# mohammadasim98/mv-ldm

Measured on AMD Instinct MI355X. Metric: denoised views/sec @ 256x256, 4 views, 50 DDIM steps, higher is better.
Workload: dtype bf16

## Files before the change

include/mvldm.h:

```cpp
#ifndef MVLDM_H
#define MVLDM_H

#include <stddef.h>
#include <stdint.h>

#ifdef __cplusplus
extern "C" {
#endif

#define MVLDM_ABI_VERSION 7

typedef void* mvldm_stream_t;

enum { MVLDM_F32 = 0, MVLDM_BF16 = 1, MVLDM_F16 = 2 };
enum { MVLDM_OK = 0, MVLDM_ERR_ARG = -1, MVLDM_ERR_HIP = -2, MVLDM_ERR_UNSUPPORTED = -3 };

enum { MVLDM_EPI_NONE = 0, MVLDM_EPI_SILU = 1, MVLDM_EPI_GEGLU = 2, MVLDM_EPI_GELU = 3  };
enum { MVLDM_ELT_COPY = 0, MVLDM_ELT_SILU = 1, MVLDM_ELT_GELU = 2 };

int mvldm_abi_version(void);
int mvldm_build_flags(void);
const char* mvldm_last_error(void);
int mvldm_device_info(int* cu_count, size_t* hbm_bytes, char* arch, int arch_len);

typedef struct mvldm_igemm_desc {
    const void* src0;
    const void* src1;
    const void* weight;
    const float* bias;
    const float* row_bias;
    const void* residual;
    void* dst;
    float* workspace;
    int32_t c0, c1;
    int32_t n_img, h_in, w_in, h_out, w_out;
    int32_t ksize, stride, pad, upsample;
    int32_t n_out, n_pad, k_pad;
    int32_t row_bias_ld;
    int32_t epilogue;
    int32_t act_dtype;
    int32_t dst_dtype;
    int32_t splitk;
    int32_t tile;
    int32_t k_order;
    int32_t dst_ld;
    float out_scale;
    size_t workspace_bytes;
} mvldm_igemm_desc;
int mvldm_igemm_fwd(const mvldm_igemm_desc* d, mvldm_stream_t stream);
size_t mvldm_igemm_workspace_bytes(const mvldm_igemm_desc* d);

int mvldm_pack_weight(const float* src, void* dst, int n_out, int c_in, int ksize, int c_pad, int n_pad,
                      int k_pad, int geglu, int k_order, int dst_dtype, int transpose, int c_off, int n_rows,
                      mvldm_stream_t stream);

int mvldm_pack_skinny(const void* packed, void* dst, int n_pad, int k_pad, int geglu, int dtype, mvldm_stream_t stream);
int mvldm_igemm_skinny_config(const mvldm_igemm_desc* d);

typedef struct mvldm_pack_job {
    const float* src; void* dst;
    int n_out, c_in, ksize, c_pad, n_pad, k_pad, geglu, k_order, transpose, c_off, n_rows;
    int kind;
    int blocks;
    int block0;
} mvldm_pack_job;
int mvldm_pack_job_prepare(mvldm_pack_job* job , int dst_dtype);
int mvldm_pack_weight_batch(const mvldm_pack_job* jobs , int n_jobs, const int32_t* block_job, int total_blocks,
                            int dst_dtype, mvldm_stream_t stream);

#define MVLDM_GN_MAX_CHUNKS 32
int mvldm_groupnorm_fwd(const void* x0, const void* x1, void* y, const float* gamma, const float* beta, int n_img,
                        int hw, int c0, int c1, int groups, float eps, int silu, int dtype, void* stats_ws,
                        float* stats_out, mvldm_stream_t stream);
int mvldm_groupnorm_passes(int n_img, int hw, int c, int groups, int dtype);

int mvldm_layernorm_fwd(const void* x, void* y, const float* gamma, const float* beta, int rows, int c, float eps,
                        int dtype, mvldm_stream_t stream);

int mvldm_attention_fwd(const void* q, const void* k, const void* v, void* out, int ld_q, int ld_k, int ld_v,
                        int ld_o, int heads, int head_dim, const int32_t* seg, int n_seg, int max_q_len,
                        float scale, int dtype, float* lse, int lse_ld, mvldm_stream_t stream);

int mvldm_timestep_embed_fwd(const int64_t* timesteps, const float* freqs, void* out, int n, int dim,
                             int flip_sin_to_cos, int dst_dtype, mvldm_stream_t stream);

int mvldm_eltwise_fwd(const void* x, void* y, size_t n, int op, int src_dtype, int dst_dtype, mvldm_stream_t stream);

int mvldm_ddim_cfg_step(const float* eps, const float* x_t, float* x_next, const int32_t* cond_img,
                        const int32_t* uncond_img, int n_tgt, int hw, int c, float cfg_scale, const float* coef,
                        const int32_t* step_ptr, void* unet_in, int unet_in_c, int unet_in_dtype, int n_steps,
                        float clip_range, mvldm_stream_t stream);
int mvldm_ddpm_cfg_step(const float* eps_c, const float* eps_u, const float* x_t, const float* noise, float* x_next, size_t n,
                        float cfg_scale, const float* coef, float clip_range, mvldm_stream_t stream);
int mvldm_ddim_advance(int32_t* step_ptr, const int64_t* t_table, int n_steps, int64_t* timesteps,
                       const int32_t* tgt_rows, int n_rows, mvldm_stream_t stream);

int mvldm_nchw_to_nhwc(const float* src, void* dst, int n_img, int c, int hw, int dst_c, int dst_c_off,
                       int dst_dtype, float scale, float shift, const int32_t* img_map, mvldm_stream_t stream);
int mvldm_nhwc_to_nchw(const void* src, float* dst, int n_img, int c, int hw, int src_c, int src_c_off,
                       int src_dtype, float scale, float shift, int clamp01, mvldm_stream_t stream);
// ... 214 lines not shown
```

mv_ldm_amd/_lib.py:

```python
from __future__ import annotations

import ctypes as C
from pathlib import Path

LIB_PATH = Path(__file__).resolve().parent / "csrc" / "libmvldm_hip.so"

ABI_VERSION = 7
F32, BF16, F16 = 0, 1, 2
EPI_NONE, EPI_SILU, EPI_GEGLU, EPI_GELU = 0, 1, 2, 3
RAYS_RAW, RAYS_POSITIONAL, RAYS_SRT = 0, 1, 2
ELT_COPY, ELT_SILU, ELT_GELU = 0, 1, 2
NORM_BWD_STORE = 0x100
GN_MAX_CHUNKS = 32

(OP_IGEMM, OP_GROUPNORM, OP_LAYERNORM, OP_ATTENTION, OP_TIMESTEP_EMBED, OP_ELTWISE, OP_DDIM_STEP, OP_DDIM_ADVANCE,
 OP_NCHW_TO_NHWC, OP_NHWC_TO_NCHW, OP_MEMCPY, OP_RAY_ENCODE, OP_POSTERIOR_SAMPLE,
 OP_WGRAD, OP_ATTENTION_BWD, OP_GROUPNORM_BWD, OP_LAYERNORM_BWD, OP_COLSUM, OP_TRAIN_ELTWISE, OP_POOL2X2, OP_ZERO_INSERT,
 OP_ADD_NOISE, OP_MSE_LOSS, OP_FILL_ZERO, OP_PAR_BEGIN, OP_PAR_NEXT, OP_PAR_END, OP_GATHER_ROWS, OP_ATTN_MERGE) = range(1, 30)
TE_SILU_BWD, TE_ADD, TE_GEGLU_FWD, TE_GEGLU_BWD, TE_GELU_BWD = 0, 1, 2, 3, 4

vp, i32, f32, sz = C.c_void_p, C.c_int32, C.c_float, C.c_size_t


class IgemmDesc(C.Structure):
    _fields_ = [("src0", vp), ("src1", vp), ("weight", vp), ("bias", vp), ("row_bias", vp), ("residual", vp),
                ("dst", vp), ("workspace", vp),
                ("c0", i32), ("c1", i32),
                ("n_img", i32), ("h_in", i32), ("w_in", i32), ("h_out", i32), ("w_out", i32),
                ("ksize", i32), ("stride", i32), ("pad", i32), ("upsample", i32),
                ("n_out", i32), ("n_pad", i32), ("k_pad", i32),
                ("row_bias_ld", i32), ("epilogue", i32), ("act_dtype", i32), ("dst_dtype", i32),
                ("splitk", i32), ("tile", i32), ("k_order", i32), ("dst_ld", i32), ("out_scale", f32), ("workspace_bytes", sz)]


class _GroupNorm(C.Structure):
    _fields_ = [("x", vp), ("x1", vp), ("y", vp), ("gamma", vp), ("beta", vp), ("stats_ws", vp),
                ("n_img", i32), ("hw", i32), ("c0", i32), ("c1", i32), ("groups", i32), ("silu", i32), ("dtype", i32),
                ("eps", f32), ("stats_out", vp)]


class _LayerNorm(C.Structure):
    _fields_ = [("x", vp), ("y", vp), ("gamma", vp), ("beta", vp), ("rows", i32), ("c", i32), ("dtype", i32), ("eps", f32)]


class _Attention(C.Structure):
    _fields_ = [("q", vp), ("k", vp), ("v", vp), ("out", vp), ("seg", vp),
                ("ld_q", i32), ("ld_k", i32), ("ld_v", i32), ("ld_o", i32), ("heads", i32), ("head_dim", i32),
                ("n_seg", i32), ("max_q_len", i32), ("dtype", i32), ("scale", f32), ("lse", vp), ("lse_ld", i32)]


class _Temb(C.Structure):
    _fields_ = [("timesteps", vp), ("freqs", vp), ("out", vp), ("n", i32), ("dim", i32), ("flip", i32), ("dst_dtype", i32)]


class _Eltwise(C.Structure):
    _fields_ = [("x", vp), ("y", vp), ("n", sz), ("op", i32), ("src_dtype", i32), ("dst_dtype", i32)]


class _Ddim(C.Structure):
    _fields_ = [("eps", vp), ("x_t", vp), ("x_next", vp), ("cond_img", vp), ("uncond_img", vp), ("coef", vp),
                ("step_ptr", vp), ("unet_in", vp),
                ("n_tgt", i32), ("hw", i32), ("c", i32), ("unet_in_c", i32), ("unet_in_dtype", i32), ("cfg_scale", f32),
                ("n_steps", i32), ("clip_range", f32)]


class _Advance(C.Structure):
    _fields_ = [("step_ptr", vp), ("t_table", vp), ("timesteps", vp), ("tgt_rows", vp), ("n_steps", i32), ("n_rows", i32)]


class _Layout(C.Structure):
    _fields_ = [("src", vp), ("dst", vp), ("n_img", i32), ("c", i32), ("hw", i32), ("other_c", i32),
                ("other_c_off", i32), ("dtype", i32), ("clamp01", i32), ("scale", f32), ("shift", f32), ("img_map", vp)]


class _Rays(C.Structure):
    _fields_ = [("extrinsics", vp), ("intrinsics", vp), ("out_nchw", vp), ("out_nhwc", vp), ("img_map", vp),
                ("n_cam", i32), ("h", i32), ("w", i32), ("nhwc_c", i32), ("nhwc_c_off", i32), ("nhwc_dtype", i32),
                ("mode", i32), ("n_origin_octaves", i32), ("n_dir_octaves", i32), ("plucker", i32)]


class _Posterior(C.Structure):
    _fields_ = [("moments", vp), ("noise", vp), ("out", vp), ("n", i32), ("c", i32), ("hw", i32), ("scale", f32)]


class _Memcpy(C.Structure):
# ... 221 lines not shown
```

mv_ldm_amd/csrc/igemm.hip:

```cpp
#include <algorithm>
#include <cstdio>
#include <cstdlib>

#include "igemm_common.h"

namespace mvldm {

template <typename T> __global__ __launch_bounds__(256) void igemm_splitk_reduce(const IgemmParams p) {
    const bool geglu = p.epilogue == MVLDM_EPI_GEGLU;
    const size_t total = (size_t)p.M * p.n_dst;
    const size_t slab = (size_t)p.M * p.n_pad;
    for (size_t idx = (size_t)blockIdx.x * 256 + threadIdx.x; idx < total; idx += (size_t)gridDim.x * 256) {
        const int m = (int)(idx / p.n_dst), col = (int)(idx - (size_t)m * p.n_dst);
        float v;
        if (geglu) {
            const int nv = (col >> 5) * 64 + (col & 31), ng = nv + 32;
            float a = 0.f, g = 0.f;
            for (int s = 0; s < p.splitk; ++s) {
                a += p.ws[s * slab + (size_t)m * p.n_pad + nv];
                g += p.ws[s * slab + (size_t)m * p.n_pad + ng];
            }
            if (p.bias) { a += p.bias[col]; g += p.bias[p.n_dst + col]; }
            v = a * gelu_erf_fast(g);
        } else {
// ... 57 lines not shown
#pragma unroll
            for (int e = 0; e < 8; ++e) a[e] += p.bias[col + e];
        }
        if (geglu) {
#pragma unroll
            for (int e = 0; e < 8; ++e) a[e] *= gelu_erf_fast(g[e] + (p.bias ? p.bias[p.n_dst + col + e] : 0.f));
        } else {
            if (p.row_bias) {
                const float* rb = p.row_bias + (size_t)(m / p.hw_out) * p.row_bias_ld + col;
#pragma unroll
                for (int e = 0; e < 8; ++e) a[e] += rb[e];
            }
            if (p.epilogue == MVLDM_EPI_SILU) {
#pragma unroll
                for (int e = 0; e < 8; ++e) a[e] = silu_f(a[e]);
            } else if (p.epilogue == MVLDM_EPI_GELU) {
#pragma unroll
                for (int e = 0; e < 8; ++e) a[e] = gelu_erf_fast(a[e]);
            }
        }
#pragma unroll
        for (int e = 0; e < 8; ++e) a[e] *= p.out_scale;
        if (p.residual) {
            const Chunk<T> rc = load_chunk<T>(reinterpret_cast<const T*>(p.residual) + (size_t)m * p.n_dst + col);
#pragma unroll
            for (int e = 0; e < 8; ++e) a[e] += rc.get(e);
        }
        size_t drow = (size_t)m;
        if (p.scatter) {
            const int img = m / p.hw_out, rem = m - img * p.hw_out;
            const int i = rem / p.w_out, j = rem - i * p.w_out;
            drow = ((size_t)img * (2 * p.h_out) + 2 * i + p.ph_y) * (size_t)(2 * p.w_out) + 2 * j + p.ph_x;
        }
        Chunk<T> oc;
#pragma unroll
        for (int e = 0; e < 8; ++e) oc.set(e, a[e]);
        store_chunk<T>(reinterpret_cast<T*>(p.dst) + drow * p.dst_ld + col, oc);
    }
}

static int env_int(const char* name, int dflt) { return knob_int(name, dflt); }
static const int kEnvTarget = env_int("MVLDM_IGEMM_TARGET", 0);
static const int kEnvSync = env_int("MVLDM_IGEMM_SYNC", 0);
static const int kEnvPx = env_int("MVLDM_IGEMM_PX", 0);
static const int kEnvNoStage = env_int("MVLDM_IGEMM_NOSTAGE", 0);
#ifdef MVLDM_EXPERIMENTS
static const int kEnvFake = env_int("MVLDM_IGEMM_FAKE", 0);
#else
static constexpr int kEnvFake = 0;
#endif

static thread_local int t_force_sync = 0;

static int launch_igemm(const IgemmParams& p, int tile, int act_dtype, hipStream_t s) {
    if (tile >= 1 && tile <= 5) return igemm_launch_small(p, tile, act_dtype, s);
    if (tile >= 6 && tile <= 8) return igemm_launch_large(p, tile, act_dtype, s);
    if (tile == 9 || tile == 10 || tile == 18) return igemm_launch_xl(p, tile, act_dtype, s);
    if (tile == 11 || tile == 17) return igemm_launch_halo(p, tile, act_dtype, s);
    return set_error(MVLDM_ERR_ARG, "igemm: bad tile %d", tile);
}


static void choose_config(const mvldm_igemm_desc& d, int M, int k_tiles, int& tile, int& splitk, size_t ws_bytes) {
    const int target = kEnvTarget ? kEnvTarget : 512;
    if (tile == 0) {
        const bool can10 = d.act_dtype != MVLDM_F32 && d.k_order == 1 && d.dst_dtype != MVLDM_F32 && d.n_pad % 320 == 0 &&
                           d.epilogue != MVLDM_EPI_GEGLU && d.upsample != 1 && d.n_out % 8 == 0 && (d.dst_ld <= 0 || d.dst_ld % 8 == 0) &&
                           !(d.ksize == 3 && d.src1);
        const int wgs10 = cdiv(M, 256) * (d.n_pad / 320);
        const double eff10 = (double)wgs10 / (256.0 * cdiv(wgs10, 256));
        if (can10 && (wgs10 >= 1024 || (wgs10 >= 512 && (eff10 >= 0.9 || d.ksize == 1)))) tile = 10;
        else if (M <= 32) tile = 5;
        else if (M <= 64) tile = 4;
        else if (d.ksize >= 2) tile = cdiv(M, 256) * cdiv(d.n_pad, 128) >= 300 ? 7 : 2;
        else if (d.n_pad >= 768 && d.act_dtype != MVLDM_F32 && d.k_order == 1 && d.dst_dtype != MVLDM_F32 &&
                 cdiv(M, 256) * cdiv(d.n_pad, 256) >= 1024)
            tile = 9;
        else if (d.k_pad >= 1024 && d.n_pad >= 1024 && cdiv(M, 128) * cdiv(d.n_pad, 256) >= 300) tile = 8;
        else tile = d.n_pad < 640 ? 2 : 3;
    }
    const int tm = cdiv(M, kTiles[tile].bm), tn = cdiv(d.n_pad, kTiles[tile].bn);
    if (splitk == 0) {
        splitk = 1;
        const int wgs = tm * tn;
        if (wgs < target) splitk = std::min(std::max(k_tiles / 4, 1), cdiv(target, wgs));
        if (d.workspace == nullptr) splitk = 1;
        while (splitk > 1 && (size_t)splitk * M * d.n_pad * sizeof(float) > ws_bytes) --splitk;
    }
    splitk = std::max(1, std::min(splitk, k_tiles));
}

static int fill_params(const mvldm_igemm_desc& d, IgemmParams& p, int& tile) {
    const int epc = d.act_dtype == MVLDM_F32 ? 4 : 8;
    const int bk = d.act_dtype == MVLDM_F32 ? 32 : 64;
    MVLDM_REQUIRE(d.src0 && d.weight && d.dst, "igemm: null pointer");
    const bool phase = d.upsample >= 2;
    MVLDM_REQUIRE(d.upsample >= 0 && d.upsample <= 5, "igemm: upsample %d", d.upsample);
    MVLDM_REQUIRE(phase ? (d.ksize == 2 && d.stride == 1 && d.h_out == d.h_in && d.w_out == d.w_in && !d.src1 && !d.residual &&
                           !d.row_bias && d.act_dtype != MVLDM_F32 && d.dst_dtype == d.act_dtype && d.k_order == 1)
                        : (d.ksize == 1 || d.ksize == 3),
                  "igemm: ksize %d / upsample %d", d.ksize, d.upsample);
    MVLDM_REQUIRE(d.stride == 1 || d.stride == 2, "igemm: stride %d", d.stride);
    MVLDM_REQUIRE(d.c0 % epc == 0 && d.c1 % epc == 0 && d.c0 > 0, "igemm: channels (%d,%d) must be multiples of %d", d.c0, d.c1, epc);
    MVLDM_REQUIRE((d.c1 == 0) == (d.src1 == nullptr), "igemm: src1/c1 mismatch");
    MVLDM_REQUIRE(d.k_pad % bk == 0 && d.k_pad >= d.ksize * d.ksize * (d.c0 + d.c1), "igemm: k_pad %d", d.k_pad);
    MVLDM_REQUIRE(d.n_pad % 64 == 0 && d.n_pad >= d.n_out, "igemm: n_pad %d (n_out %d)", d.n_pad, d.n_out);
    MVLDM_REQUIRE(d.dst_dtype == d.act_dtype || d.dst_dtype == MVLDM_F32, "igemm: dst dtype");
    if (d.epilogue == MVLDM_EPI_GEGLU)
        MVLDM_REQUIRE(d.n_out % 64 == 0 && !d.row_bias, "igemm: GEGLU needs n_out %% 64 == 0");
    p.src0 = d.src0; p.src1 = d.src1; p.weight = d.weight; p.bias = d.bias; p.row_bias = d.row_bias;
    p.residual = d.residual; p.dst = d.dst; p.ws = d.workspace;
    p.c0 = d.c0; p.c1 = d.c1; p.ctot = d.c0 + d.c1;
    p.n_img = d.n_img; p.h_in = d.h_in; p.w_in = d.w_in; p.h_out = d.h_out; p.w_out = d.w_out;
    p.hw_out = d.h_out * d.w_out;
    p.ksize = d.ksize; p.stride = d.stride; p.pad = d.pad; p.upsample = phase ? 0 : d.upsample; p.taps = d.ksize * d.ksize;
    p.scatter = phase; p.ph_y = phase ? (d.upsample - 2) >> 1 : 0; p.ph_x = phase ? (d.upsample - 2) & 1 : 0;
    p.ty0 = phase ? p.ph_y - 1 : -d.pad; p.tx0 = phase ? p.ph_x - 1 : -d.pad;
    p.cy = phase ? 1 - p.ph_y : d.ksize / 2; p.cx = phase ? 1 - p.ph_x : d.ksize / 2;
    p.M = d.n_img * p.hw_out; p.n_out = d.n_out; p.n_pad = d.n_pad; p.k_pad = d.k_pad;
    p.n_dst = d.epilogue == MVLDM_EPI_GEGLU ? d.n_out / 2 : d.n_out;
    p.rb_vec = d.row_bias && ((uintptr_t)d.row_bias % 16 == 0) && d.row_bias_ld % 4 == 0;
    p.bias_vec = d.bias && ((uintptr_t)d.bias % 16 == 0);
    p.row_bias_ld = d.row_bias_ld; p.epilogue = d.epilogue; p.dst_f32 = d.dst_dtype == MVLDM_F32;
    p.out_scale = d.out_scale;
    p.dst_ld = d.dst_ld > 0 ? d.dst_ld : p.n_dst;
    MVLDM_REQUIRE(p.dst_ld >= p.n_dst, "igemm: dst_ld %d < n_dst %d", p.dst_ld, p.n_dst);
    p.k_tiles = d.k_pad / bk;
    tile = d.tile & 63;
    t_force_sync = (d.tile >> 12) & 1;
    const int force_px = (d.tile >> 8) & 15;
    int splitk = d.splitk;
    MVLDM_REQUIRE(((tile >= 0 && tile <= kNumTiles) || tile == 17 || deep_tile(tile)) && splitk >= 0, "igemm: tile/splitk");
    choose_config(d, p.M, p.k_tiles, tile, splitk, d.workspace_bytes);
    if (splitk > 1)
        MVLDM_REQUIRE(d.workspace && (size_t)splitk * p.M * d.n_pad * sizeof(float) <= d.workspace_bytes,
                      "igemm: split-K workspace too small");
    const double es = 2.0;
    const double b0 = (double)d.n_img * d.h_in * d.w_in * d.c0 * es, b1 = (double)d.n_img * d.h_in * d.w_in * d.c1 * es;
    const double bw = (double)d.n_pad * d.k_pad * es;
    p.use_bl = d.act_dtype != MVLDM_F32 && d.k_order == 1 && !t_force_sync && !kEnvSync &&
               b0 < 4.0e9 && b1 < 4.0e9 && bw < 4.0e9;
    if (d.act_dtype != MVLDM_F32 && d.k_order == 1 && !t_force_sync && !kEnvSync && !p.use_bl) {
        static bool warned = false;
        if (!warned) {
            warned = true;
            fprintf(stderr, "[mvldm] igemm: operand of %.2f GB exceeds the 4 GB range of the fast 16-bit loop; using the slower "
                            "64-bit-address loop (split the batch to avoid this)\n", std::max(std::max(b0, b1), bw) / 1e9);
        }
    }
    p.src0_bytes = (unsigned)b0; p.src1_bytes = (unsigned)b1; p.w_bytes = (unsigned)bw;
    p.fake = kEnvFake;
    p.nt_store = stream_stores((size_t)p.M * (size_t)p.n_dst * (p.dst_f32 || d.act_dtype == MVLDM_F32 ? 4 : 2));
    if (kEnvFake & 1) p.src0_bytes = p.src1_bytes = 0;
    if (kEnvFake & 2) p.w_bytes = 0;
    if (tile >= 6 && !p.use_bl) tile = 2;
    if (deep_tile(tile) && d.upsample) tile = 2;
    p.splitk = splitk;
    if (p.use_bl) {
        const int cbs = p.k_tiles / p.taps;
        const int per = cdiv(cbs, std::min(splitk, cbs));
        p.k_tiles_per_split = per * p.taps;
        p.splitk = cdiv(cbs, per);
    } else {
        p.k_tiles_per_split = cdiv(p.k_tiles, splitk);
        p.splitk = cdiv(p.k_tiles, p.k_tiles_per_split);
    }
    p.stage_epi = d.act_dtype != MVLDM_F32 && !kEnvNoStage && (p.splitk > 1 || (!p.dst_f32 && p.n_dst % 8 == 0 && p.dst_ld % 8 == 0));
    if (tile >= 9 && tile <= 10 && (!p.stage_epi || (tile == 10 && d.epilogue == MVLDM_EPI_GEGLU))) tile = 7;
    if (tile == 11 && !(p.use_bl && p.stage_epi && p.splitk == 1 && d.ksize == 3 && d.stride == 1 && d.pad == 1 && !d.upsample &&
                        d.h_out == d.h_in && d.w_out == d.w_in && halo_rows_for(d.w_in) <= 384 && halo_smem(d.w_in) <= 160 * 1024))
        tile = 7;
    if (tile == 17 && !(p.use_bl && p.stage_epi && p.splitk == 1 && d.ksize == 3 && d.stride == 1 && d.pad == 1 && !d.upsample && d.c1 == 0 &&
                        d.h_out == d.h_in && d.w_out == d.w_in && d.epilogue != MVLDM_EPI_GEGLU && halow_smem(d.w_in) <= 160 * 1024))
        tile = 7;
    if (phase) {
        MVLDM_REQUIRE(p.use_bl && p.stage_epi, "igemm: 2x2 phase conv needs the lean 16-bit loop and an 8-aligned 16-bit output");
        if (tile != 7 && tile != 10) tile = 2;
    }
    if (p.use_bl && d.upsample == 1 && tile != 7) tile = 2;
    if (p.use_bl && d.upsample != 1) {
        const int hc = (d.h_out - 1) * d.stride + p.ty0 + p.cy, wc = (d.w_out - 1) * d.stride + p.tx0 + p.cx;
        MVLDM_REQUIRE(p.ty0 + p.cy >= 0 && p.tx0 + p.cx >= 0 && hc < d.h_in && wc < d.w_in,
                      "igemm: conv geometry (pad %d, stride %d) not supported", d.pad, d.stride);
    }
    p.tiles_m = cdiv(p.M, kTiles[tile].bm);
    p.tiles_n = cdiv(d.n_pad, kTiles[tile].bn);
    p.korder = d.k_order;
    if (d.k_order)
        MVLDM_REQUIRE(d.k_order == 1 && p.ctot % bk == 0 && d.c0 % bk == 0 && d.k_pad == p.taps * p.ctot,
                      "igemm: k_order 1 needs channel counts (%d,%d) multiples of %d", d.c0, d.c1, bk);
    {
        const double a_bytes = (double)d.n_img * d.h_in * d.w_in * p.ctot, w_bytes = (double)d.n_pad * d.k_pad;
        double best = 1e300;
        for (int px = 1; px <= 8; px *= 2) {
            const int py = 8 / px;
            const int sm = cdiv(p.tiles_m, px), sn = cdiv(p.tiles_n, py);
            const double waste = (double)(8 * sm * sn) / ((double)p.tiles_m * p.tiles_n);
            const double cost = (py * a_bytes + px * w_bytes) * waste * waste;
            if (cost < best) { best = cost; p.px = px; p.sub_m = sm; p.sub_n = sn; }
        }
        p.m_fast = w_bytes >= a_bytes;
        const int fpx = force_px ? force_px : kEnvPx;
        if (fpx > 0 && fpx <= 8 && (8 % fpx) == 0) {
            p.px = fpx; p.sub_m = cdiv(p.tiles_m, p.px); p.sub_n = cdiv(p.tiles_n, 8 / p.px);
        }
        p.grp_m = p.grp_n = 1;
        static const int kGroup = knob_int("MVLDM_IGEMM_GROUP", -1);
        if (kGroup != 0 && ((tile >= 7 && tile <= 10) || tile == 17) && p.sub_m * p.sub_n > 32) {
            const double ax = a_bytes / p.px, wx = w_bytes / (8 / p.px);
            double bestc = 1e300;
            for (int gm = 1; gm <= 32; gm *= 2) {
                if (kGroup > 0 && gm != kGroup) continue;
                const int gme = std::min(gm, p.sub_m), gne = std::min(32 / gm, p.sub_n);
                const double c = ax * cdiv(p.sub_n, gne) + wx * cdiv(p.sub_m, gme);
                if (c < bestc) { bestc = c; p.grp_m = gme; p.grp_n = gne; }
            }
        }
    }
    return MVLDM_OK;
}

int linear_pp_run(const mvldm_igemm_desc& d, hipStream_t s);
int linear_pw_run(const mvldm_igemm_desc& d, hipStream_t s);
int linear_ws_run(const mvldm_igemm_desc& d, hipStream_t s);
int skinny_run(const mvldm_igemm_desc& d, hipStream_t s);
int linear_rs_run(const mvldm_igemm_desc& d, hipStream_t s);

int igemm_run(const mvldm_igemm_desc& d, hipStream_t s) {
    IgemmParams p;
    int tile = 0;
    if (d.n_img == 0 || d.h_out == 0 || d.w_out == 0) return MVLDM_OK;
    const int req = d.tile & 63;
    if (req == 15) return skinny_run(d, s);
    if (req == 12 || req == 13 || req == 14 || req == 19) {
        MVLDM_REQUIRE(d.src0 && d.weight && d.dst, "igemm: null pointer");
        return req == 12 ? linear_pp_run(d, s) : req == 13 ? linear_pw_run(d, s) : req == 14 ? linear_ws_run(d, s) : linear_rs_run(d, s);
    }
    MVLDM_REQUIRE(d.k_order != 2, "igemm: the fragment-order pack (k_order 2) is read by tile 15 only");
    int rc = fill_params(d, p, tile);
    if (rc) return rc;
    if (p.M == 0) return MVLDM_OK;
    rc = dispatch_dtype(d.act_dtype, [&](auto t) {
        using T = decltype(t);
        int r = launch_igemm(p, tile, Elt<T>::DT, s);
        if (r) return r;
        if (p.splitk > 1) {
            if constexpr (sizeof(T) == 2) {
                if (!p.dst_f32 && p.n_dst % 8 == 0 && p.dst_ld % 8 == 0 && ((uintptr_t)p.ws % 16) == 0 &&
                    (!p.residual || ((uintptr_t)p.residual % 16) == 0) && ((uintptr_t)p.dst % 16) == 0) {
                    const size_t chunks = (size_t)p.M * (p.n_dst / 8);
                    hipLaunchKernelGGL(igemm_splitk_reduce_vec<T>, dim3((unsigned)std::min<size_t>((chunks + 255) / 256, 4096)), dim3(256), 0, s, p);
                    return check_launch();
                }
            }
            const size_t total = (size_t)p.M * p.n_dst;
            const int blocks = (int)std::min<size_t>((total + 255) / 256, 4096);
            hipLaunchKernelGGL(igemm_splitk_reduce<T>, dim3(blocks), dim3(256), 0, s, p);
            return check_launch();
        }
        return (int)MVLDM_OK;
    });
    return rc;
}

}

using namespace mvldm;

extern "C" int mvldm_igemm_fwd(const mvldm_igemm_desc* d, mvldm_stream_t stream) {
    MVLDM_REQUIRE(d != nullptr, "igemm: null desc");
    return igemm_run(*d, (hipStream_t)stream);
}

extern "C" size_t mvldm_igemm_workspace_bytes(const mvldm_igemm_desc* d) {
    if (!d) return 0;
    const size_t M = (size_t)d->n_img * d->h_out * d->w_out;
    return (size_t)16 * M * d->n_pad * sizeof(float);
}
```

mv_ldm_amd/csrc/igemm_bl.h:

```cpp
#pragma once
#include "igemm_common.h"

namespace mvldm {

template <typename T, int BM, int BN, int WM, int WN>
__global__ __launch_bounds__(WM* WN * 64) void igemm_kernel(const IgemmParams p) {
    using M_ = Mma<T>;
    constexpr int NT = WM * WN * 64;
    constexpr int EPC = Elt<T>::EPC;
    constexpr int BK = M_::BK;
    constexpr int TM = BM / WM / 32, TN = BN / WN / 32;
    constexpr int A_BYTES = BM * M_::PITCH, B_BYTES = BN * M_::PITCH;
    constexpr int A_IT = BM * 8 / NT, B_IT = BN * 8 / NT;
    static_assert(A_IT >= 1 && B_IT >= 1 && TM >= 1 && TN >= 1, "bad tile");
    extern __shared__ __attribute__((aligned(16))) char smem[];

    const int tid = threadIdx.x, lane = tid & 63, wave = tid >> 6;
    const int wm = wave / WN, wn = wave % WN;
    const int hi = lane >> 5, l31 = lane & 31;

    int split, tm, tn;
    if (!map_block(p, split, tm, tn)) return;
    const int kt0 = split * p.k_tiles_per_split;
    const int kt1 = min(kt0 + p.k_tiles_per_split, p.k_tiles);

    const int kc = tid & 7, r0 = tid >> 3;
    int a_img[A_IT], a_y[A_IT], a_x[A_IT];
#pragma unroll
    for (int it = 0; it < A_IT; ++it) {
        const int m = tm * BM + r0 + it * (NT / 8);
        if (m < p.M) {
            const int img = m / p.hw_out, rem = m - img * p.hw_out;
            const int oy = rem / p.w_out;
            a_img[it] = img;
            a_y[it] = oy * p.stride - p.pad;
            a_x[it] = (rem - oy * p.w_out) * p.stride - p.pad;
        } else {
            a_img[it] = -1; a_y[it] = 0; a_x[it] = 0;
        }
    }
    const T* wbase = reinterpret_cast<const T*>(p.weight) + (size_t)(tn * BN + r0) * p.k_pad + kc * EPC;
    const int hs = p.upsample ? 2 * p.h_in : p.h_in, wsz = p.upsample ? 2 * p.w_in : p.w_in;

    u32x4 areg[A_IT], breg[B_IT];
    auto load_tile = [&](int kt) {
        int tap, c;
        if (p.korder) {
            const int cb = kt / p.taps;
            tap = kt - cb * p.taps;
            c = cb * BK + kc * EPC;
        } else {
            const int ke = kt * BK + kc * EPC;
            tap = ke / p.ctot;
            c = ke - tap * p.ctot;
        }
        const bool tap_ok = tap < p.taps;
        const int ky = tap / p.ksize, kx = tap - ky * p.ksize;
        const bool from0 = c < p.c0;
        const T* sbase = from0 ? reinterpret_cast<const T*>(p.src0) + c
// ... 32 lines not shown
    f32x16 acc[TM][TN];
#pragma unroll
    for (int i = 0; i < TM; ++i)
#pragma unroll
        for (int j = 0; j < TN; ++j)
#pragma unroll
            for (int r = 0; r < 16; ++r) acc[i][j][r] = 0.f;

    if (kt0 < kt1) {
        load_tile(kt0);
        store_tile(0);
    }
    __syncthreads();
    int cur = 0;
    for (int kt = kt0; kt < kt1; ++kt) {
        const bool more = kt + 1 < kt1;
        if (more) load_tile(kt + 1);
        const char* at = smem + cur * (A_BYTES + B_BYTES);
        const char* bt = at + A_BYTES;
#pragma unroll
        for (int kk = 0; kk < BK / M_::KI; ++kk) {
            typename M_::Frag a[TM], b[TN];
#pragma unroll
            for (int i = 0; i < TM; ++i) a[i] = M_::load(at, wm * (BM / WM) + i * 32 + l31, kk, hi);
#pragma unroll
            for (int j = 0; j < TN; ++j) b[j] = M_::load(bt, wn * (BN / WN) + j * 32 + l31, kk, hi);
#pragma unroll
            for (int i = 0; i < TM; ++i)
#pragma unroll
                for (int j = 0; j < TN; ++j) acc[i][j] = M_::mma(a[i], b[j], acc[i][j]);
        }
        if (more) store_tile(cur ^ 1);
        __syncthreads();
        cur ^= 1;
    }

    if constexpr (sizeof(T) == 2) {
        if (p.stage_epi) {
            igemm_epilogue_staged<T, BM, BN, WM, WN>(p, acc, tm, tn, split, wm, wn, wave, lane, smem);
            return;
        }
    }
    igemm_epilogue<T, BM, BN, WM, WN>(p, acc, tm, tn, split, wm, wn, hi, l31);
}


template <int TAPS, int A_IT, bool DUAL, bool UPS> struct BlAddr {
    unsigned a0[UPS ? TAPS : 1][A_IT];
    unsigned a1[DUAL ? (UPS ? TAPS : 1) : 1][DUAL ? A_IT : 1];
    unsigned mask[UPS ? 1 : A_IT];
};

template <typename T, int BM, int BN, int NW, int KS, bool DUAL, int A_IT, int B_IT, int STAGES, bool UPS, int t, int LO = 0, int HI = 1 << 20>
__device__ __forceinline__ void bl_issue(const IgemmParams& p, char* stage_base, int wave, int cb,
                                         const BlAddr<KS * KS, A_IT, DUAL, UPS>& ad, const unsigned (&vb)[B_IT]) {
    constexpr int BK = 64, TAPS = KS * KS;
    const int lead = (!UPS && KS > 1) ? p.w_in + 1 : 0;
    const int disp = UPS ? 0 : (t / KS - p.cy) * p.w_in + (t % KS - p.cx) + lead;
    const unsigned lead0 = (unsigned)lead * (unsigned)p.c0 * 2u, lead1 = (unsigned)lead * (unsigned)p.c1 * 2u;
    const __amdgpu_buffer_rsrc_t r0 = __builtin_amdgcn_make_buffer_rsrc(
        const_cast<char*>(reinterpret_cast<const char*>(p.src0)) - lead0, 0, p.src0_bytes + lead0, 0x00020000);
    const __amdgpu_buffer_rsrc_t r1 = __builtin_amdgcn_make_buffer_rsrc(
        const_cast<char*>(reinterpret_cast<const char*>(DUAL ? p.src1 : p.src0)) - (DUAL ? lead1 : lead0), 0,
        DUAL ? p.src1_bytes + lead1 : p.src0_bytes + lead0, 0x00020000);
    const __amdgpu_buffer_rsrc_t rw = __builtin_amdgcn_make_buffer_rsrc(const_cast<void*>(p.weight), 0, p.w_bytes, 0x00020000);
    char* at = stage_base;
    char* bt = at + BM * 128;
    const int c = cb * BK;
    const bool from0 = !DUAL || c < p.c0;
    const int soff = ((from0 ? c : c - p.c0) + disp * (from0 ? p.c0 : p.c1)) * 2;
#pragma unroll
    for (int it = (LO > 0 ? LO : 0); it < (HI < A_IT ? HI : A_IT); ++it) {
        __attribute__((address_space(3))) void* dst = (__attribute__((address_space(3))) void*)(at + (wave + NW * it) * 1024);
        unsigned v0, v1;
        if constexpr (UPS) {
            v0 = ad.a0[t][it];
            v1 = ad.a1[DUAL ? t : 0][DUAL ? it : 0];
        } else {
            const bool ok = (ad.mask[it] >> t) & 1u;
            v0 = ok ? ad.a0[0][it] : kBufOob;
            v1 = ok ? ad.a1[0][DUAL ? it : 0] : kBufOob;
        }
        if (from0) __builtin_amdgcn_raw_ptr_buffer_load_lds(r0, dst, 16, v0, soff, 0, 0);
        else __builtin_amdgcn_raw_ptr_buffer_load_lds(r1, dst, 16, v1, soff, 0, 0);
    }
    const int koff = (cb * TAPS + t) * (BK * 2);
#pragma unroll
    for (int it = (LO > A_IT ? LO - A_IT : 0); it < (HI - A_IT < B_IT ? HI - A_IT : B_IT); ++it)
        __builtin_amdgcn_raw_ptr_buffer_load_lds(rw, (__attribute__((address_space(3))) void*)(bt + (wave + NW * it) * 1024), 16,
                                                 vb[it], koff, 0, 0);
}

template <typename T, int BM, int BN, int WM, int WN>
__device__ __forceinline__ void bl_compute(const char* stage_base, f32x16 (&acc)[BM / WM / 32][BN / WN / 32], int wm, int wn,
                                           int hi, int l31) {
    constexpr int TM = BM / WM / 32, TN = BN / WN / 32;
#pragma unroll
    for (int kk = 0; kk < 64 / Mma<T>::KI; ++kk) {
        BlFrags<T, TM, TN> f;
        bl_load<T, BM, BN, WM, WN>(stage_base, f, kk, wm, wn, hi, l31);
        bl_mma<T, TM, TN>(f, acc);
    }
}

template <int LPT, int MAXY>
__device__ __forceinline__ void bl_wait_young(int young) {
    if constexpr (MAXY >= 1) {
        if (young >= MAXY) {
            asm volatile("s_waitcnt vmcnt(%0) lgkmcnt(0)" ::"n"(MAXY * LPT) : "memory");
            return;
        }
        bl_wait_young<LPT, MAXY - 1>(young);
    } else {
        asm volatile("s_waitcnt vmcnt(0) lgkmcnt(0)" ::: "memory");
    }
}

template <typename T, int BM, int BN, int WM, int WN, int KS, bool DUAL, int STAGES, bool UPS>
__global__ __launch_bounds__(WM* WN * 64) void igemm_bl_kernel(const IgemmParams p) {
    using M_ = Mma<T>;
    static_assert(sizeof(T) == 2, "16-bit activation types only");
    constexpr int NW = WM * WN, TAPS = KS * KS;
    constexpr int BK = 64, EPC = 8;
    constexpr int TM = BM / WM / 32, TN = BN / WN / 32;
    constexpr int A_BYTES = BM * 128, B_BYTES = BN * 128, STAGE_BYTES = A_BYTES + B_BYTES;
    constexpr int A_IT = BM / 8 / NW, B_IT = BN / 8 / NW, LPT = A_IT + B_IT;
    static_assert(A_IT >= 1 && B_IT >= 1 && (BM / 8) % NW == 0 && (BN / 8) % NW == 0, "bad tile");
    static_assert(STAGES >= 2 && STAGES <= 8, "ring depth");
    extern __shared__ __attribute__((aligned(16))) char smem[];

    const auto [lane, wave, wm, wn, hi, l31] = wave_lane<WN>();
    int split, tm, tn;
    if (!map_block(p, split, tm, tn)) return;
    const int cb0 = split * (p.k_tiles_per_split / TAPS);
    const int cb1 = min(cb0 + p.k_tiles_per_split / TAPS, p.k_tiles / TAPS);

    const int slot = lane & 7, rsub = lane >> 3;
    BlAddr<TAPS, A_IT, DUAL, UPS> ad;
#pragma unroll
    for (int it = 0; it < A_IT; ++it) {
        const int row = (wave + NW * it) * 8 + rsub;
        const int m = tm * BM + row;
        const unsigned chunk = (unsigned)((slot ^ ((row >> 1) & 7)) * EPC);
        const bool live = m < p.M;
        const int img = live ? m / p.hw_out : 0, rem = live ? m - img * p.hw_out : 0;
        const int oy = rem / p.w_out, ox = rem - oy * p.w_out;
        if constexpr (UPS) {
            const unsigned hs = 2 * p.h_in, wsz = 2 * p.w_in;
            const int y0 = live ? oy * p.stride - p.pad : -(1 << 20), x0 = ox * p.stride - p.pad;
#pragma unroll
            for (int t = 0; t < TAPS; ++t) {
                const int iy = y0 + t / KS, ix = x0 + t % KS;
                const bool ok = (unsigned)iy < hs && (unsigned)ix < wsz;
                const unsigned pix = (unsigned)(img * p.h_in + (iy >> 1)) * (unsigned)p.w_in + (unsigned)(ix >> 1);
                ad.a0[t][it] = ok ? (pix * (unsigned)p.c0 + chunk) * 2u : kBufOob;
                if constexpr (DUAL) ad.a1[t][it] = ok ? (pix * (unsigned)p.c1 + chunk) * 2u : kBufOob;
            }
        } else {
            const int yc = oy * p.stride + p.ty0 + p.cy, xc = ox * p.stride + p.tx0 + p.cx;
            const unsigned pix = (unsigned)(img * p.h_in + yc) * (unsigned)p.w_in + (unsigned)xc;
            unsigned msk = 0;
#pragma unroll
            for (int t = 0; t < TAPS; ++t) {
                const int iy = yc + t / KS - p.cy, ix = xc + t % KS - p.cx;
                msk |= (live && (unsigned)iy < (unsigned)p.h_in && (unsigned)ix < (unsigned)p.w_in) ? (1u << t) : 0u;
            }
            ad.a0[0][it] = (pix * (unsigned)p.c0 + chunk) * 2u;
            if constexpr (DUAL) ad.a1[0][it] = (pix * (unsigned)p.c1 + chunk) * 2u;
            ad.mask[it] = msk;
        }
    }
    unsigned vb[B_IT];
// ... 124 lines not shown
        if (cb0 < cb1) {
            MVLDM_BL_ISSUE(0, cb0, 0);
            int slot_c = 0;
            for (int cb = cb0; cb < cb1; ++cb) {
                MVLDM_BL_STEP_SIMPLE(0)
                if constexpr (TAPS == 4) { MVLDM_BL_STEP_SIMPLE(1) MVLDM_BL_STEP_SIMPLE(2) MVLDM_BL_STEP_SIMPLE(3) }
                if constexpr (TAPS == 9) {
                    MVLDM_BL_STEP_SIMPLE(1) MVLDM_BL_STEP_SIMPLE(2) MVLDM_BL_STEP_SIMPLE(3) MVLDM_BL_STEP_SIMPLE(4)
                    MVLDM_BL_STEP_SIMPLE(5) MVLDM_BL_STEP_SIMPLE(6) MVLDM_BL_STEP_SIMPLE(7) MVLDM_BL_STEP_SIMPLE(8)
                }
            }
        }
    } else if (cb0 < cb1) {
        MVLDM_BL_ISSUE(0, cb0, 0);
        const bool has1 = cb0 + 1 / TAPS < cb1, has2 = STAGES == 3 && cb0 + 2 / TAPS < cb1;
        if (has1) { MVLDM_BL_ISSUE(1, cb0 + 1 / TAPS, (1 % TAPS)); }
        if constexpr (STAGES == 3) {
            if (has2) { MVLDM_BL_ISSUE(2, cb0 + 2 / TAPS, (2 % TAPS)); }
        }
        if (has2) asm volatile("s_waitcnt vmcnt(%0)" ::"n"(2 * LPT) : "memory");
        else if (has1) asm volatile("s_waitcnt vmcnt(%0)" ::"n"(LPT) : "memory");
        else asm volatile("s_waitcnt vmcnt(0)" ::: "memory");
        __builtin_amdgcn_s_barrier();
        int slot_c = 0;
        BlFrags<T, TM, TN> f0, f1;
        MVLDM_BL_LOAD(f0, 0, 0);
        for (int cb = cb0; cb < cb1; ++cb) {
            MVLDM_BL_STEP(0)
            if constexpr (TAPS == 4) { MVLDM_BL_STEP(1) MVLDM_BL_STEP(2) MVLDM_BL_STEP(3) }
            if constexpr (TAPS == 9) {
                MVLDM_BL_STEP(1) MVLDM_BL_STEP(2) MVLDM_BL_STEP(3) MVLDM_BL_STEP(4)
                MVLDM_BL_STEP(5) MVLDM_BL_STEP(6) MVLDM_BL_STEP(7) MVLDM_BL_STEP(8)
            }
        }
    }
#undef MVLDM_BL_STEP_SIMPLE
#undef MVLDM_BL_STEP_DEEP
#undef MVLDM_BL_PRO
#undef MVLDM_BL_LOAD
#undef MVLDM_BL_MMA
#undef MVLDM_BL_NEXT
#undef MVLDM_BL_STEP
#undef MVLDM_BL_ISSUE
#undef MVLDM_BL_ISSUE_R
    asm volatile("s_waitcnt vmcnt(0)" ::: "memory");
    if constexpr (TM * TN > 4) {
        igemm_epilogue_staged<T, BM, BN, WM, WN>(p, acc, tm, tn, split, wm, wn, wave, lane, smem);
    } else {
        if (p.stage_epi) igemm_epilogue_staged<T, BM, BN, WM, WN>(p, acc, tm, tn, split, wm, wn, wave, lane, smem);
        else igemm_epilogue<T, BM, BN, WM, WN>(p, acc, tm, tn, split, wm, wn, hi, l31);
    }
}

template <typename T, int BM, int BN, int WM, int WN> static int launch_sync(const IgemmParams& p, hipStream_t s) {
    static std::atomic<uint64_t> done{0};
    constexpr int ring = 2 * (BM + BN) * Mma<T>::PITCH, park = WM * WN * 32 * (park_blocks(BN / WN / 32) * 32 + 4) * 4;
    return launch_kernel(igemm_kernel<T, BM, BN, WM, WN>, done, (sizeof(T) == 2 && park > ring) ? park : ring,
                         8 * p.sub_m * p.sub_n * p.splitk, WM * WN * 64, p, s);
}

template <typename T, int BM, int BN, int WM, int WN, int KS, bool DUAL, int STAGES, bool UPS>
static int launch_bl_s(const IgemmParams& p, hipStream_t s) {
    static std::atomic<uint64_t> done{0};
    constexpr int ring = STAGES * (BM + BN) * 128, park = WM * WN * 32 * (park_blocks(BN / WN / 32) * 32 + 4) * 4;
    return launch_kernel(igemm_bl_kernel<T, BM, BN, WM, WN, KS, DUAL, STAGES, UPS>, done, ring > park ? ring : park,
                         8 * p.sub_m * p.sub_n * p.splitk, WM * WN * 64, p, s);
}
template <typename T, int BM, int BN, int WM, int WN, int KS, bool DUAL, int DEPTH = 0>
static int launch_bl(const IgemmParams& p, hipStream_t s) {
    constexpr int STAGES = DEPTH ? DEPTH : ((WM * WN == 8 && 3 * (BM + BN) * 128 <= 160 * 1024) ? 3 : 2);
    if (p.upsample) {
        if constexpr (KS == 3 && !DUAL && ((BM == 128 && BN == 64) || (BM == 256 && BN == 128)))
            return launch_bl_s<T, BM, BN, WM, WN, KS, DUAL, STAGES, true>(p, s);
        else
            return set_error(MVLDM_ERR_ARG, "igemm: upsampling 3x3 conv needs tile 2 or 7 on the 16-bit path");
    }
    return launch_bl_s<T, BM, BN, WM, WN, KS, DUAL, STAGES, false>(p, s);
}
template <typename T, int BM, int BN, int WM, int WN, int DEPTH> static int launch_bl_deep(const IgemmParams& p, hipStream_t s) {
    const bool dual = p.c1 > 0;
    if (p.ksize == 3) return dual ? launch_bl<T, BM, BN, WM, WN, 3, true, DEPTH>(p, s) : launch_bl<T, BM, BN, WM, WN, 3, false, DEPTH>(p, s);
    if (p.ksize == 1) return dual ? launch_bl<T, BM, BN, WM, WN, 1, true, DEPTH>(p, s) : launch_bl<T, BM, BN, WM, WN, 1, false, DEPTH>(p, s);
    return set_error(MVLDM_ERR_ARG, "igemm: the deep-ring tiles take 1x1 and 3x3 convs");
}

template <typename T, int BM, int BN, int WM, int WN> static int launch_bl_any(const IgemmParams& p, hipStream_t s) {
    const bool dual = p.c1 > 0;
    if (p.ksize == 2) {
        if constexpr ((BM == 128 && BN == 64) || (BM == 256 && BN == 128) || (BM == 256 && BN == 320))
            return launch_bl<T, BM, BN, WM, WN, 2, false>(p, s);
        else
            return set_error(MVLDM_ERR_ARG, "igemm: 2x2 phase conv needs tile 2, 7 or 10");
    }
    if (p.ksize == 3) {
        if (!dual) return launch_bl<T, BM, BN, WM, WN, 3, false>(p, s);
        if constexpr (BM == 256 && BN >= 256)
            return set_error(MVLDM_ERR_UNSUPPORTED, "igemm: tiles 9 / 10 do not take a two-source 3x3 conv (use tile 7 or 11)");
        else
            return launch_bl<T, BM, BN, WM, WN, 3, true>(p, s);
    }
    return dual ? launch_bl<T, BM, BN, WM, WN, 1, true>(p, s) : launch_bl<T, BM, BN, WM, WN, 1, false>(p, s);
}

template <typename T, int BM, int BN, int WM, int WN> static int launch_tile(const IgemmParams& p, hipStream_t s) {
    if constexpr (sizeof(T) == 2) {
        if (p.use_bl) return launch_bl_any<T, BM, BN, WM, WN>(p, s);
    }
    return launch_sync<T, BM, BN, WM, WN>(p, s);
}

}
```

mv_ldm_amd/csrc/igemm_common.h:

```cpp
#pragma once
#include <algorithm>

#include "common.h"

namespace mvldm {

struct IgemmParams {
    const void* src0; const void* src1; const void* weight;
    const float* bias; const float* row_bias; const void* residual; void* dst; float* ws;
    int c0, c1, ctot;
    int n_img, h_in, w_in, h_out, w_out, hw_out;
    int ksize, stride, pad, upsample;
    int M, n_out, n_pad, n_dst, k_pad, taps;
    int row_bias_ld, epilogue, dst_f32, dst_ld;
    float out_scale;
    int splitk, k_tiles, k_tiles_per_split;
    int tiles_m, tiles_n;
    int korder;
    int px, sub_m, sub_n, m_fast;
    int grp_m, grp_n;
    int rb_vec;
    int bias_vec;
    int ty0, tx0, cy, cx;
    int scatter, ph_y, ph_x;
    int fake;
    unsigned src0_bytes, src1_bytes, w_bytes;
    int use_bl, stage_epi;
    int nt_store;
};

template <typename T> struct Mma;

template <typename T16> struct Mma16 : Mfma16<T16> {
    static constexpr int KI = 16;
    static constexpr int BK = 64;
    static constexpr int PITCH = 128;
    using Frag = typename Mfma16<T16>::Frag;
    static __device__ __forceinline__ void store(char* tile, int r, int kc, u32x4 v) {
        *reinterpret_cast<u32x4*>(tile + r * PITCH + ((kc ^ ((r >> 1) & 7)) << 4)) = v;
    }
    static __device__ __forceinline__ Frag load(const char* tile, int r, int kk, int hi) {
        const int kc = kk * 2 + hi;
        return *reinterpret_cast<const Frag*>(tile + r * PITCH + ((kc ^ ((r >> 1) & 7)) << 4));
    }
};
template <> struct Mma<bf16_t> : Mma16<bf16_t> {};
template <> struct Mma<f16_t> : Mma16<f16_t> {};
template <> struct Mma<float> {
    static constexpr int KI = 2;
    static constexpr int BK = 32;
    static constexpr int PITCH = 33 * 4;
    using Frag = float;
    static __device__ __forceinline__ void store(char* tile, int r, int kc, u32x4 v) {
        uint32_t* p = reinterpret_cast<uint32_t*>(tile + r * PITCH + kc * 16);
        p[0] = v[0]; p[1] = v[1]; p[2] = v[2]; p[3] = v[3];
    }
    static __device__ __forceinline__ Frag load(const char* tile, int r, int kk, int hi) {
        return *reinterpret_cast<const float*>(tile + r * PITCH + (kk * 2 + hi) * 4);
    }
    static __device__ __forceinline__ f32x16 mma(Frag a, Frag b, f32x16 c) {
        return __builtin_amdgcn_mfma_f32_32x32x2f32(a, b, c, 0, 0, 0);
    }
};

__device__ __forceinline__ int orig_col(int n_packed, int n_out, bool geglu) {
    if (!geglu) return n_packed;
    const int blk = n_packed >> 5, w = n_packed & 31;
    return (blk & 1) ? (n_out >> 1) + (blk >> 1) * 32 + w : (blk >> 1) * 32 + w;
}

template <typename T, bool SCATTER = false>
__device__ __forceinline__ void epilogue_store(const IgemmParams& p, int m, int n_dst_col, float v) {
    v *= p.out_scale;
    if (p.residual) v += to_f32<T>(reinterpret_cast<const T*>(p.residual)[(size_t)m * p.n_dst + n_dst_col]);
    size_t drow = (size_t)m;
    if (SCATTER && p.scatter) {
        const int img = m / p.hw_out, rem = m - img * p.hw_out;
        const int i = rem / p.w_out, j = rem - i * p.w_out;
        drow = ((size_t)img * (2 * p.h_out) + 2 * i + p.ph_y) * (size_t)(2 * p.w_out) + 2 * j + p.ph_x;
    }
    const size_t o = drow * p.dst_ld + n_dst_col;
    if (p.dst_f32) reinterpret_cast<float*>(p.dst)[o] = v;
    else reinterpret_cast<T*>(p.dst)[o] = from_f32<T>(v);
}

__device__ __forceinline__ bool map_block(const IgemmParams& p, int& split, int& tm, int& tn) {
    const int b = blockIdx.x, xcd = b & 7, idx = b >> 3;
    const int xm = xcd % p.px, xn = xcd / p.px;
    const int per = p.sub_m * p.sub_n;
    split = idx / per;
    const int r = idx - split * per;
    int tml, tnl;
    if (p.grp_m * p.grp_n > 1) {
        const int gm = p.grp_m, gn = p.grp_n;
        const int nfull = p.sub_m / gm, per_super = gm * p.sub_n;
        int mg, gm_eff, rr;
        if (r < nfull * per_super) { mg = r / per_super; rr = r - mg * per_super; gm_eff = gm; }
        else { mg = nfull; rr = r - nfull * per_super; gm_eff = p.sub_m - nfull * gm; }
        const int ng = rr / (gm_eff * gn), r2 = rr - ng * gm_eff * gn;
        tnl = ng * gn + r2 / gm_eff;
        tml = mg * gm + r2 % gm_eff;
    } else if (p.m_fast) { tnl = r / p.sub_m; tml = r - tnl * p.sub_m; }
    else { tml = r / p.sub_n; tnl = r - tml * p.sub_n; }
    tm = xm * p.sub_m + tml;
    tn = xn * p.sub_n + tnl;
    return tm < p.tiles_m && tn < p.tiles_n;
}

template <typename T, int BM, int BN, int WM, int WN>
__device__ __forceinline__ void igemm_epilogue(const IgemmParams& p, f32x16 (&acc)[BM / WM / 32][BN / WN / 32], int tm, int tn,
                                               int split, int wm, int wn, int hi, int l31) {
    constexpr int TM = BM / WM / 32, TN = BN / WN / 32;
    const bool geglu = p.epilogue == MVLDM_EPI_GEGLU;
    if (p.splitk > 1) {
        float* ws = p.ws + (size_t)split * p.M * p.n_pad;
#pragma unroll
        for (int i = 0; i < TM; ++i)
#pragma unroll
            for (int j = 0; j < TN; ++j) {
                const int n = tn * BN + wn * (BN / WN) + j * 32 + l31;
#pragma unroll
                for (int r = 0; r < 16; ++r) {
                    const int m = tm * BM + wm * (BM / WM) + i * 32 + (r & 3) + 8 * (r >> 2) + 4 * hi;
                    if (m < p.M && n < p.n_pad) ws[(size_t)m * p.n_pad + n] = acc[i][j][r];
                }
            }
        return;
    }
#pragma unroll
    for (int i = 0; i < TM; ++i) {
        if (geglu) {
            if constexpr (TN % 2 == 0) {
#pragma unroll
                for (int j = 0; j < TN; j += 2) {
                    const int nb = tn * BN + wn * (BN / WN) + j * 32;
                    const int col = (nb >> 6) * 32 + l31;
                    if (col >= p.n_dst) continue;
                    const float bv = p.bias ? p.bias[col] : 0.f;
                    const float bg = p.bias ? p.bias[p.n_dst + col] : 0.f;
#pragma unroll
                    for (int r = 0; r < 16; ++r) {
                        const int m = tm * BM + wm * (BM / WM) + i * 32 + (r & 3) + 8 * (r >> 2) + 4 * hi;
                        if (m >= p.M) continue;
                        epilogue_store<T>(p, m, col, (acc[i][j][r] + bv) * gelu_erf_fast(acc[i][j + 1][r] + bg));
                    }
                }
            }
        } else {
#pragma unroll
            for (int j = 0; j < TN; ++j) {
                const int n = tn * BN + wn * (BN / WN) + j * 32 + l31;
                if (n >= p.n_out) continue;
                const float bv = p.bias ? p.bias[n] : 0.f;
#pragma unroll
                for (int r = 0; r < 16; ++r) {
                    const int m = tm * BM + wm * (BM / WM) + i * 32 + (r & 3) + 8 * (r >> 2) + 4 * hi;
                    if (m >= p.M) continue;
                    float v = acc[i][j][r] + bv;
                    if (p.row_bias) v += p.row_bias[(size_t)(m / p.hw_out) * p.row_bias_ld + n];
                    if (p.epilogue == MVLDM_EPI_SILU) v = silu_f(v);
                    else if (p.epilogue == MVLDM_EPI_GELU) v = gelu_erf_fast(v);
                    epilogue_store<T>(p, m, n, v);
                }
            }
        }
    }
}

constexpr int park_blocks(int tn) { return tn <= 4 ? tn : 4; }

enum { EPI_PLAIN = 0, EPI_ACT_SILU = 1, EPI_PAIR_GEGLU = 2, EPI_PARTIAL = 3, EPI_ACT_GELU = 4 };

template <typename T, int JN, int MODE, int PITCH>
__device__ __forceinline__ void epi_rows(const IgemmParams& p, const float* st, int m0, int pcol0, int split, int lane) {
    constexpr bool PAIR = MODE == EPI_PAIR_GEGLU;
    constexpr int WC = PAIR ? JN * 16 : JN * 32;
    constexpr int CPR = WC / 8;
    static_assert(64 % CPR == 0 && (32 * CPR) % 64 == 0, "row-major mapping");
    constexpr int RSTEP = 64 / CPR, ITERS = 32 / RSTEP;
    const int ch = lane % CPR, row0 = lane / CPR;
    const int ncol0 = PAIR ? (pcol0 >> 1) : pcol0;
    const int n0 = ncol0 + ch * 8;
    const int n_lim = MODE == EPI_PARTIAL ? p.n_pad : p.n_dst;
    if (n0 >= n_lim) return;
    const int voff = PAIR ? (2 * (ch >> 2)) * 32 + (ch & 3) * 8 : ch * 8;
    float bv[8], bg[8];
#pragma unroll
    for (int e = 0; e < 8; ++e) bv[e] = bg[e] = 0.f;
    if (MODE != EPI_PARTIAL && p.bias) {
        if (p.bias_vec) {
            const f32x4 b0 = *reinterpret_cast<const f32x4*>(p.bias + n0), b1 = *reinterpret_cast<const f32x4*>(p.bias + n0 + 4);
#pragma unroll
            for (int e = 0; e < 4; ++e) { bv[e] = b0[e]; bv[4 + e] = b1[e]; }
            if constexpr (PAIR) {
                const f32x4 g0 = *reinterpret_cast<const f32x4*>(p.bias + p.n_dst + n0);
                const f32x4 g1 = *reinterpret_cast<const f32x4*>(p.bias + p.n_dst + n0 + 4);
#pragma unroll
                for (int e = 0; e < 4; ++e) { bg[e] = g0[e]; bg[4 + e] = g1[e]; }
            }
        } else {
#pragma unroll
            for (int e = 0; e < 8; ++e) {
                bv[e] = p.bias[n0 + e];
                if constexpr (PAIR) bg[e] = p.bias[p.n_dst + n0 + e];
            }
        }
    }
    const bool rb_on = MODE != EPI_PARTIAL && MODE != EPI_PAIR_GEGLU && p.row_bias != nullptr;
    Chunk<T> rpre[ITERS];
    if constexpr (MODE != EPI_PARTIAL) {
        if (p.residual && !(p.fake & 4)) {
#pragma unroll
            for (int it = 0; it < ITERS; ++it) {
                const int m = m0 + row0 + it * RSTEP;
                if (m < p.M) rpre[it] = load_chunk<T>(reinterpret_cast<const T*>(p.residual) + (size_t)m * p.n_dst + n0);
            }
        }
    }
    float rbv[8];
    bool rb_pre = false;
    if (rb_on) {
        const int img0 = m0 / p.hw_out;
        rb_pre = p.rb_vec && (min(m0 + 31, p.M - 1) / p.hw_out) == img0;
        if (rb_pre) {
            const float* rb = p.row_bias + (size_t)img0 * p.row_bias_ld + n0;
            const f32x4 r0 = *reinterpret_cast<const f32x4*>(rb), r1 = *reinterpret_cast<const f32x4*>(rb + 4);
#pragma unroll
            for (int e = 0; e < 4; ++e) { rbv[e] = r0[e]; rbv[4 + e] = r1[e]; }
        }
    }
#pragma unroll
    for (int it = 0; it < ITERS; ++it) {
        const int row = row0 + it * RSTEP;
        const int m = m0 + row;
        if (m >= p.M) continue;
        const f32x4 a = *reinterpret_cast<const f32x4*>(st + row * PITCH + voff);
        const f32x4 b = *reinterpret_cast<const f32x4*>(st + row * PITCH + voff + 4);
        if constexpr (MODE == EPI_PARTIAL) {
            float* o = p.ws + (size_t)split * p.M * p.n_pad + (size_t)m * p.n_pad + n0;
            *reinterpret_cast<f32x4*>(o) = a;
            *reinterpret_cast<f32x4*>(o + 4) = b;
        } else {
            float v[8] = {a[0] + bv[0], a[1] + bv[1], a[2] + bv[2], a[3] + bv[3], b[0] + bv[4], b[1] + bv[5], b[2] + bv[6], b[3] + bv[7]};
            if constexpr (PAIR) {
                const f32x4 ga = *reinterpret_cast<const f32x4*>(st + row * PITCH + voff + 32);
                const f32x4 gb = *reinterpret_cast<const f32x4*>(st + row * PITCH + voff + 36);
#pragma unroll
                for (int e = 0; e < 4; ++e) {
                    v[e] *= gelu_erf_16(ga[e] + bg[e]);
                    v[4 + e] *= gelu_erf_16(gb[e] + bg[4 + e]);
                }
            } else {
                if (rb_on && rb_pre) {
#pragma unroll
                    for (int e = 0; e < 8; ++e) v[e] += rbv[e];
                } else if (rb_on) {
                    const float* rb = p.row_bias + (size_t)(m / p.hw_out) * p.row_bias_ld + n0;
                    if (p.rb_vec) {
                        const f32x4 r0 = *reinterpret_cast<const f32x4*>(rb), r1 = *reinterpret_cast<const f32x4*>(rb + 4);
#pragma unroll
                        for (int e = 0; e < 4; ++e) { v[e] += r0[e]; v[4 + e] += r1[e]; }
                    } else {
#pragma unroll
                        for (int e = 0; e < 8; ++e) v[e] += rb[e];
                    }
                }
                if constexpr (MODE == EPI_ACT_SILU) {
#pragma unroll
                    for (int e = 0; e < 8; ++e) v[e] = silu_f(v[e]);
                }
                if constexpr (MODE == EPI_ACT_GELU) {
#pragma unroll
                    for (int e = 0; e < 8; ++e) v[e] = gelu_erf_fast(v[e]);
                }
            }
#pragma unroll
            for (int e = 0; e < 8; ++e) v[e] *= p.out_scale;
            if (p.fake & 4) { if (v[0] == 1.2345e33f) p.ws[0] = v[1]; continue; }
            if (p.residual) {
#pragma unroll
                for (int e = 0; e < 8; ++e) v[e] += rpre[it].get(e);
            }
            Chunk<T> oc;
#pragma unroll
            for (int e = 0; e < 8; ++e) oc.set(e, v[e]);
            size_t drow = (size_t)m;
            if (p.scatter) {
                const int img = m / p.hw_out, rem = m - img * p.hw_out;
                const int i = rem / p.w_out, j = rem - i * p.w_out;
                drow = ((size_t)img * (2 * p.h_out) + 2 * i + p.ph_y) * (size_t)(2 * p.w_out) + 2 * j + p.ph_x;
            }
            T* const dptr = reinterpret_cast<T*>(p.dst) + drow * p.dst_ld + n0;
            if (p.nt_store) __builtin_nontemporal_store(oc.raw, reinterpret_cast<u32x4*>(dptr));
            else store_chunk<T>(dptr, oc);
        }
    }
}

template <int TM, int TN, int I, int J0, int JN, int PITCH>
__device__ __forceinline__ void epi_park(const f32x16 (&acc)[TM][TN], float* st, int lane) {
    const int hi = lane >> 5, l31 = lane & 31;
#pragma unroll
    for (int j = 0; j < JN; ++j)
#pragma unroll
        for (int r = 0; r < 16; ++r) st[((r & 3) + 8 * (r >> 2) + 4 * hi) * PITCH + j * 32 + l31] = acc[I][J0 + j][r];
}

template <typename T, int JN, int PITCH>
__device__ __forceinline__ void epi_group_rows(const IgemmParams& p, const float* st, int m0, int pcol0, int split, int mode, int lane) {
    if (mode == EPI_PARTIAL) epi_rows<T, JN, EPI_PARTIAL, PITCH>(p, st, m0, pcol0, split, lane);
    else if (mode == EPI_PAIR_GEGLU) {
        if constexpr (JN % 2 == 0) epi_rows<T, JN, EPI_PAIR_GEGLU, PITCH>(p, st, m0, pcol0, split, lane);
    } else if (mode == EPI_ACT_SILU) epi_rows<T, JN, EPI_ACT_SILU, PITCH>(p, st, m0, pcol0, split, lane);
    else if (mode == EPI_ACT_GELU) epi_rows<T, JN, EPI_ACT_GELU, PITCH>(p, st, m0, pcol0, split, lane);
    else epi_rows<T, JN, EPI_PLAIN, PITCH>(p, st, m0, pcol0, split, lane);
}

template <typename T, int BM, int BN, int WM, int WN, int I>
__device__ __forceinline__ void igemm_epilogue_rowblock(const IgemmParams& p, const f32x16 (&acc)[BM / WM / 32][BN / WN / 32], float* st, int tm, int tn,
                                                        int split, int wm, int wn, int mode, int lane) {
    constexpr int TM = BM / WM / 32, TN = BN / WN / 32;
    constexpr int WCOLS = BN / WN;
    constexpr int JG = park_blocks(TN);
    constexpr int PITCH = JG * 32 + 4;
    const int m0 = tm * BM + wm * (BM / WM) + I * 32;
    const int pcol0 = tn * BN + wn * WCOLS;
    epi_park<TM, TN, I, 0, JG, PITCH>(acc, st, lane);
    epi_group_rows<T, JG, PITCH>(p, st, m0, pcol0, split, mode, lane);
    if constexpr (TN > JG) {
        epi_park<TM, TN, I, JG, TN - JG, PITCH>(acc, st, lane);
        epi_group_rows<T, TN - JG, PITCH>(p, st, m0, pcol0 + JG * 32, split, mode, lane);
    }
    if constexpr (I + 1 < TM) igemm_epilogue_rowblock<T, BM, BN, WM, WN, I + 1>(p, acc, st, tm, tn, split, wm, wn, mode, lane);
}

template <typename T, int BM, int BN, int WM, int WN>
__device__ __forceinline__ void igemm_epilogue_staged(const IgemmParams& p, f32x16 (&acc)[BM / WM / 32][BN / WN / 32], int tm,
                                                      int tn, int split, int wm, int wn, int wave, int lane, char* smem) {
    constexpr int TN = BN / WN / 32;
    constexpr int JG = park_blocks(TN);
    constexpr int PITCH = JG * 32 + 4;
    static_assert(TN <= 2 * JG, "at most two park groups");
    if (p.fake & 8) return;
    float* st = reinterpret_cast<float*>(smem) + wave * (32 * PITCH);
    const int mode = p.splitk > 1 ? EPI_PARTIAL
                                  : (p.epilogue == MVLDM_EPI_GEGLU ? EPI_PAIR_GEGLU
                                     : (p.epilogue == MVLDM_EPI_SILU ? EPI_ACT_SILU : (p.epilogue == MVLDM_EPI_GELU ? EPI_ACT_GELU : EPI_PLAIN)));
    __syncthreads();
    igemm_epilogue_rowblock<T, BM, BN, WM, WN, 0>(p, acc, st, tm, tn, split, wm, wn, mode, lane);
}

struct WaveLane { int lane, wave, wm, wn, hi, l31; };
template <int WN> __device__ __forceinline__ WaveLane wave_lane() {
    const int tid = threadIdx.x, lane = tid & 63;
    const int wave = __builtin_amdgcn_readfirstlane(tid >> 6);
    return {lane, wave, wave / WN, wave % WN, lane >> 5, lane & 31};
}

template <typename T, int TM, int TN> struct BlFrags {
    typename Mma<T>::Frag a[TM], b[TN];
};

template <typename T, int BM, int BN, int WM, int WN>
__device__ __forceinline__ void bl_load(const char* stage_base, BlFrags<T, BM / WM / 32, BN / WN / 32>& f, int kk, int wm, int wn,
                                        int hi, int l31) {
    using M_ = Mma<T>;
    constexpr int TM = BM / WM / 32, TN = BN / WN / 32;
    const char* at = stage_base;
    const char* bt = at + BM * 128;
#pragma unroll
    for (int i = 0; i < TM; ++i) f.a[i] = M_::load(at, wm * (BM / WM) + i * 32 + l31, kk, hi);
#pragma unroll
    for (int j = 0; j < TN; ++j) f.b[j] = M_::load(bt, wn * (BN / WN) + j * 32 + l31, kk, hi);
}

template <typename T, int TM, int TN>
__device__ __forceinline__ void bl_mma(const BlFrags<T, TM, TN>& f, f32x16 (&acc)[TM][TN]) {
#pragma unroll
    for (int i = 0; i < TM; ++i)
#pragma unroll
        for (int j = 0; j < TN; ++j) acc[i][j] = Mma<T>::mma(f.a[i], f.b[j], acc[i][j]);
}

inline int cdiv(int a, int b) { return (a + b - 1) / b; }
struct TileCfg { int bm, bn, threads; };
constexpr TileCfg kTiles[] = {{0, 0, 0}, {128, 128, 256}, {128, 64, 256}, {64, 128, 256}, {64, 64, 128}, {32, 64, 64},
                                 {256, 64, 256},
                                 {256, 128, 512},
                                 {128, 256, 512},
                                 {256, 256, 512},
                                 {256, 320, 512},
                                 {256, 128, 512},
                                 {0, 0, 0}, {0, 0, 0}, {0, 0, 0}, {0, 0, 0},
                                 {0, 0, 0},
                                 {256, 320, 512},
                                 {192, 128, 512}};
constexpr int kNumTiles = 11;
inline bool deep_tile(int tile) { return tile == 18; }

template <typename KernT> inline int launch_kernel(KernT kern, std::atomic<uint64_t>& attr_done, int smem, int blocks, int threads,
                                                   const IgemmParams& p, hipStream_t s) {
    if (int rc0 = ensure_dyn_smem(reinterpret_cast<const void*>(kern), smem, attr_done)) return rc0;
    hipLaunchKernelGGL(kern, dim3(blocks), dim3(threads), smem, s, p);
    return check_launch();
}

inline int halo_rows_for(int w_in) { return (256 + 2 * (w_in + 1) + 7) / 8 * 8; }
inline int halo_smem(int w_in) { return 2 * halo_rows_for(w_in) * 128 + 3 * 128 * 128 + 128 + 1024; }
inline int halow_smem(int w_in) { return 2 * halo_rows_for(w_in) * 128 + 2 * 320 * 128 + 128 + 1024; }

inline int require_bl(const IgemmParams& p, int tile, int act_dtype) {
    if (act_dtype != MVLDM_F32 && p.use_bl) return MVLDM_OK;
    return set_error(MVLDM_ERR_ARG, "igemm: tile %d needs the 16-bit block-major path", tile);
}
template <typename F> inline int dispatch_16bit(int dtype, F&& f) { return dtype == MVLDM_BF16 ? f(bf16_t{}) : f(f16_t{}); }

int igemm_launch_small(const IgemmParams& p, int tile, int act_dtype, hipStream_t s);
int igemm_launch_large(const IgemmParams& p, int tile, int act_dtype, hipStream_t s);
int igemm_launch_xl(const IgemmParams& p, int tile, int act_dtype, hipStream_t s);
int igemm_launch_halo(const IgemmParams& p, int tile, int act_dtype, hipStream_t s);

}
```

mv_ldm_amd/csrc/igemm_large.hip:

```cpp
#include "igemm_bl.h"

namespace mvldm {

int igemm_launch_large(const IgemmParams& p, int tile, int act_dtype, hipStream_t s) {
    if (int rc = require_bl(p, tile, act_dtype)) return rc;
    return dispatch_16bit(act_dtype, [&](auto t) {
        using T = decltype(t);
        switch (tile) {
            case 6: return launch_bl_any<T, 256, 64, 4, 1>(p, s);
            case 7: return launch_bl_any<T, 256, 128, 4, 2>(p, s);
            case 8: return launch_bl_any<T, 128, 256, 2, 4>(p, s);
            default: return set_error(MVLDM_ERR_ARG, "igemm: bad tile %d", tile);
        }
    });
}

}
```

mv_ldm_amd/csrc/igemm_small.hip:

```cpp
#include "igemm_bl.h"

namespace mvldm {

int igemm_launch_small(const IgemmParams& p, int tile, int act_dtype, hipStream_t s) {
    return dispatch_dtype(act_dtype, [&](auto t) {
        using T = decltype(t);
        switch (tile) {
            case 1: return launch_tile<T, 128, 128, 2, 2>(p, s);
            case 2: return launch_tile<T, 128, 64, 4, 1>(p, s);
            case 3: return launch_tile<T, 64, 128, 2, 2>(p, s);
            case 4: return launch_tile<T, 64, 64, 2, 1>(p, s);
            case 5: return launch_tile<T, 32, 64, 1, 1>(p, s);
            default: return set_error(MVLDM_ERR_ARG, "igemm: bad tile %d", tile);
        }
    });
}

}
```

mv_ldm_amd/csrc/igemm_xl.hip:

```cpp
#include "igemm_bl.h"

namespace mvldm {

int igemm_launch_xl(const IgemmParams& p, int tile, int act_dtype, hipStream_t s) {
    if (tile == 18) {
        if (p.epilogue == MVLDM_EPI_GEGLU) return set_error(MVLDM_ERR_UNSUPPORTED, "igemm: tile 18 does not take the GEGLU epilogue");
        if (act_dtype == MVLDM_F32 || !p.use_bl || p.upsample)
            return set_error(MVLDM_ERR_ARG, "igemm: tile 18 needs the 16-bit block-major path (no upsampling forms)");
    } else if (int rc = require_bl(p, tile, act_dtype)) {
        return rc;
    }
    return dispatch_16bit(act_dtype, [&](auto t) {
        using T = decltype(t);
        switch (tile) {
            case 9: return launch_bl_any<T, 256, 256, 4, 2>(p, s);
            case 10: return launch_bl_any<T, 256, 320, 4, 2>(p, s);
            case 18: return launch_bl_deep<T, 192, 128, 2, 4, 4>(p, s);
            default: return set_error(MVLDM_ERR_ARG, "igemm: bad tile %d", tile);
        }
    });
}

}
```

mv_ldm_amd/csrc/skinny.hip:

```cpp
#include <algorithm>
#include <cstdio>
#include <cstdlib>
#include <cstring>

#include "common.h"

namespace mvldm {

struct SkParams {
    const void* src0; const void* src1; const void* w;
    const float* bias; const float* row_bias; const void* residual; void* dst;
    int c0, c1;
    int n_img, h_in, w_in, hw_in, h_out, w_out, hw_out;
    int stride, ty0, tx0, ksize;
    int M, n_out, n_dst, dst_ld, row_bias_ld, rb_hw;
    int epilogue, dst_f32;
    float out_scale;
    int n_tiles;
    int n_groups, m_groups, G;
    int n_cbs, cb0;
    int n_stages;
    int ksteps;
    int scatter, ph_y, ph_x;
    int hw_sh, w_sh, rb_sh;
// ... 616 lines not shown
        }
    }
    switch (cfg) {
        case 1: return sk_launch<T, SkCfg<9, 9, 1, 3, 1, 10, 1>>(p, grid, s);
        case 2: return sk_launch<T, SkCfg<9, 9, 1, 4, 1, 10, 1>>(p, grid, s);
        case 5: return sk_launch<T, SkCfg<9, 9, 1, 3, 1, 5, 4>>(p, grid, s);
        case 6: return sk_launch<T, SkCfg<4, 8, 2, 3, 1, 5, 1>>(p, grid, s);
        case 7: return sk_launch<T, SkCfg<4, 8, 2, 4, 1, 5, 1>>(p, grid, s);
        case 8: return sk_launch<T, SkCfg<1, 8, 4, 3, 4, 5, 1>>(p, grid, s);
        case 9: return sk_launch<T, SkCfg<1, 8, 4, 3, 2, 5, 1>>(p, grid, s);
        case 10: return sk_launch<T, SkCfg<1, 8, 4, 1, 4, 5, 1>>(p, grid, s);
        case 12: return sk_launch<T, SkCfg<1, 8, 4, 3, 1, 5, 1>>(p, grid, s);
        case 13: return sk_launch<T, SkCfg<1, 4, 2, 6, 2, 5, 1>>(p, grid, s);
        case 18: return sk_launch<T, SkCfg<9, 9, 1, 12, 1, 3, 1>>(p, grid, s);
        case 19: return sk_launch<T, SkCfg<4, 8, 2, 12, 1, 3, 1>>(p, grid, s);
        case 20: return sk_launch<T, SkCfg<1, 8, 4, 1, 2, 5, 1>>(p, grid, s);
        case 38: return iw_launch<T, IwCfg<1, 4, 3, 1, 5, 1>>(p, grid, s);
        case 39: return iw_launch<T, IwCfg<1, 4, 3, 2, 5, 1>>(p, grid, s);
        case 40: return iw_launch<T, IwCfg<1, 4, 3, 4, 5, 1>>(p, grid, s);
        case 41: return iw_launch<T, IwCfg<1, 4, 1, 2, 5, 1>>(p, grid, s);
        case 42: return iw_launch<T, IwCfg<1, 4, 1, 4, 5, 1>>(p, grid, s);
        case 43: return iw_launch<T, IwCfg<1, 8, 3, 1, 2, 1>>(p, grid, s);
        case 44: return iw_launch<T, IwCfg<1, 4, 6, 2, 2, 1>>(p, grid, s);
        case 46: return iw_launch<T, IwCfg<1, 8, 3, 2, 2, 1>>(p, grid, s);
        default: return set_error(MVLDM_ERR_ARG, "igemm: tile 15: bad configuration %d", cfg);
    }
}

struct SkGeom { int n_img, h_in, w_in, h_out, w_out; };
static SkGeom sk_geom(const mvldm_igemm_desc& d) {
    if (d.ksize == 1 && d.stride == 1 && d.pad == 0 && d.h_in == d.h_out && d.w_in == d.w_out) return {d.n_img * d.h_out * d.w_out, 1, 1, 1, 1};
    return {d.n_img, d.h_in, d.w_in, d.h_out, d.w_out};
}

static bool sk_cfg_fits(const SkinnyCfgInfo& c, const mvldm_igemm_desc& d) {
    const SkGeom g = sk_geom(d);
    const int taps = d.ksize * d.ksize, hw_out = g.h_out * g.w_out, hw_in = g.h_in * g.w_in;
    if (c.taps != taps) return false;
    const int rows = c.mt * 16;
    if (hw_out > rows || rows % hw_out) return false;
    const int G = rows / hw_out;
    if (G * hw_in > rows * c.sm) return false;
    if (d.epilogue == MVLDM_EPI_GEGLU && (c.nt & 1)) return false;
    if (c.taps == 0) return false;
    if (d.c1 > 0) {
        const bool sk2 = c.sc > 0 && c.taps == 1 && ((c.nw == 8 && c.sc == 4 && (c.mt == 3 || c.mt == 1)) || (c.nw == 4 && c.mt == 6));
        const bool iw2 = c.sc == 0 && c.taps == 1 && c.nw == 4 && (c.mt == 3 || c.mt == 6) && !(c.mt == 1);
        if (!sk2 && !iw2) return false;
    }
    return true;
}

bool skinny_applicable(const mvldm_igemm_desc& d) {
    if (d.act_dtype == MVLDM_F32 || d.k_order != 2) return false;
    if (!(d.ksize == 1 || d.ksize == 3 || (d.ksize == 2 && d.upsample >= 2)) || (d.upsample == 1)) return false;
    if (d.ksize != 2 && d.upsample != 0) return false;
    if (d.c0 % 64 || d.c1 % 64 || d.c0 <= 0 || (d.c1 == 0) != (d.src1 == nullptr)) return false;
    if (d.k_pad != d.ksize * d.ksize * (d.c0 + d.c1) || d.n_pad % 64 || d.n_out % 4 || d.n_out > d.n_pad) return false;
    if (d.dst_dtype != d.act_dtype && d.dst_dtype != MVLDM_F32) return false;
    if (d.epilogue == MVLDM_EPI_GEGLU && (d.n_out % 64 || d.row_bias || d.n_out != d.n_pad)) return false;
    const int n_dst = d.epilogue == MVLDM_EPI_GEGLU ? d.n_out / 2 : d.n_out;
    const int dst_ld = d.dst_ld > 0 ? d.dst_ld : n_dst;
    if (dst_ld % 4 || dst_ld < n_dst) return false;
    if (d.bias && ((uintptr_t)d.bias % 16)) return false;
    if (d.row_bias && (((uintptr_t)d.row_bias % 16) || d.row_bias_ld % 4)) return false;
    if (((uintptr_t)d.dst % 16) || ((uintptr_t)d.weight % 16) || (d.residual && ((uintptr_t)d.residual % 8))) return false;
    if (((uintptr_t)d.src0 % 16) || (d.src1 && ((uintptr_t)d.src1 % 16))) return false;
    const double px = (double)d.n_img * d.h_in * d.w_in;
    if (px * d.c0 * 2.0 >= 4.0e9 || px * d.c1 * 2.0 >= 4.0e9 || (double)d.n_pad * d.k_pad * 2.0 >= 4.0e9) return false;
    if (d.residual && d.upsample >= 2) return false;
    return true;
}

static int sk_choose(const mvldm_igemm_desc& d) {
    const SkGeom g = sk_geom(d);
    const int hw = g.h_out * g.w_out, taps = d.ksize * d.ksize, M = g.n_img * hw;
    int pref[6] = {0, 0, 0, 0, 0, 0};
    if (taps == 9) {
        if (d.stride == 2) { pref[0] = 5; }
        else if (hw > 48) { pref[0] = g.n_img >= 2 ? 18 : 2; pref[1] = 2; pref[2] = 18; }
        else { pref[0] = 1; pref[1] = 18; pref[2] = 2; }
    } else if (taps == 4) {
        if (hw > 48) { pref[0] = g.n_img >= 2 ? 19 : 7; pref[1] = 7; pref[2] = 19; }
        else { pref[0] = 6; pref[1] = 7; pref[2] = 19; }
    } else {
        if (M <= 16) { pref[0] = 20; pref[1] = 41; pref[2] = 10; }
        else if (M <= 160) {
            if (d.n_pad >= 2560) { pref[0] = 8; pref[1] = 40; }
            else { pref[0] = 38; pref[1] = 12; }
            pref[2] = 9;
        } else {
            if (d.n_pad <= 1280) { pref[0] = 44; pref[1] = 13; pref[2] = 9; }
            else { pref[0] = 8; pref[1] = 40; }
        }
        pref[4] = 12; pref[5] = 8;
    }
    for (int c : pref)
        if (c > 0 && c < kNumSkCfgs && sk_cfg_fits(kSkCfgs[c], d)) return c;
    for (int c = 1; c < kNumSkCfgs; ++c)
        if (sk_cfg_fits(kSkCfgs[c], d)) return c;
    return 0;
}

int skinny_run(const mvldm_igemm_desc& d, hipStream_t s) {
    MVLDM_REQUIRE(d.src0 && d.weight && d.dst, "igemm: null pointer");
    MVLDM_REQUIRE(skinny_applicable(d), "igemm: tile 15 (skinny weight-streaming GEMM) does not apply to this problem (needs the fragment-order "
                                        "pack, k_order 2, 16-bit activations, channels in multiples of 64, ksize 1 / 3 or a 2x2 phase conv)");
// ... 92 lines not shown
```

mv_ldm_amd/modules.py:

```python
from __future__ import annotations

import math
import os
from types import SimpleNamespace
from typing import List, Optional, Sequence

import torch
from torch import nn

from . import _lib as L
from . import ops
from .ops import PackedWeight
from .plan import Builder
from .runtime import from_nhwc, get_compute_dtype, require_gpu, to_nhwc


_EPOCH_COUNTER = [0]


def bump_weights_epoch(module=None) -> int:
    _EPOCH_COUNTER[0] += 1
    e = _EPOCH_COUNTER[0]
    if module is None:
        _GLOBAL_FLOOR[0] = e
# ... 102 lines not shown

class Timesteps(nn.Module):

    def __init__(self, num_channels: int, flip_sin_to_cos: bool = True, downscale_freq_shift: float = 0.0):
        super().__init__()
        self.num_channels, self.flip_sin_to_cos, self.downscale_freq_shift = num_channels, flip_sin_to_cos, downscale_freq_shift
        half = num_channels // 2
        exponent = -math.log(10000) * torch.arange(0, half, dtype=torch.float32) / (half - downscale_freq_shift)
        self.register_buffer("freqs", torch.exp(exponent), persistent=False)

    def emit(self, b: Builder, timesteps, dtype=torch.float32):
        return b.timestep_embed(timesteps, self.freqs, self.num_channels, self.flip_sin_to_cos, dtype)

    def forward(self, timesteps):
        require_gpu(timesteps)
        return ops.timestep_embed(timesteps.to(torch.int64).contiguous(), self.freqs, self.num_channels,
                                  self.flip_sin_to_cos, torch.float32)


class TimestepEmbedding(nn.Module):
    def __init__(self, in_channels: int, time_embed_dim: int):
        super().__init__()
        self.linear_1 = Linear(in_channels, time_embed_dim)
        self.act = nn.SiLU()
        self.linear_2 = Linear(time_embed_dim, time_embed_dim)

    def emit(self, b: Builder, t_emb, silu_out=False):
        h = self.linear_1.emit(b, t_emb, epilogue=L.EPI_SILU, name="time_embedding.linear_1")
        out = self.linear_2.emit(b, h, epilogue=L.EPI_SILU if silu_out else L.EPI_NONE, name="time_embedding.linear_2")
        b.free(h)
        return out

    def forward(self, sample):
        b = eager_builder(sample)
        x = sample if sample.dtype == b.dtype else ops.convert(sample.contiguous(), b.dtype)
        return self.emit(b, x)


class ResnetBlock2D(nn.Module):

    def __init__(self, in_channels, out_channels=None, temb_channels=512, groups=32, eps=1e-6):
        super().__init__()
        out_channels = in_channels if out_channels is None else out_channels
        self.in_channels, self.out_channels = in_channels, out_channels
        self.norm1 = GroupNorm(groups, in_channels, eps=eps)
        self.conv1 = Conv2d(in_channels, out_channels, 3, padding=1)
        self.time_emb_proj = Linear(temb_channels, out_channels) if temb_channels is not None else None
        self.norm2 = GroupNorm(groups, out_channels, eps=eps)
        self.dropout = nn.Dropout(0.0)
        self.conv2 = Conv2d(out_channels, out_channels, 3, padding=1)
        self.nonlinearity = nn.SiLU()
        self.conv_shortcut = Conv2d(in_channels, out_channels, 1) if in_channels != out_channels else None

    def emit(self, b: Builder, x, temb=None, x2=None, temb_proj=None, out=None):
        if self.time_emb_proj is not None and temb_proj is None:
            ta = b.eltwise(temb, L.ELT_SILU, name="temb_silu")
            temb_proj = self.time_emb_proj.emit(b, ta, out_dtype=torch.float32, name="time_emb_proj")
            b.free(ta)
        def main_chain():
            g1 = self.norm1.emit(b, x, silu=True, x2=x2, name="norm1+silu")
            h = self.conv1.emit(b, g1, row_bias=temb_proj, name="conv1")
            b.free(g1)
            g2 = self.norm2.emit(b, h, silu=True, name="norm2+silu")
            b.free(h)
            return g2

        if self.conv_shortcut is None:
            assert x2 is None
            g2, sc = main_chain(), x
        elif b.small_launch(x.shape[0] * x.shape[1] * x.shape[2], self.conv_shortcut.out_channels):
            with b.parallel() as par:
                par.lane()
                g2 = main_chain()
                par.lane()
                sc = self.conv_shortcut.emit(b, x, x2=x2, name="conv_shortcut")
        else:
            g2 = main_chain()
            sc = self.conv_shortcut.emit(b, x, x2=x2, name="conv_shortcut")
        out = self.conv2.emit(b, g2, residual=sc, name="conv2", **({} if out is None else {"out": out}))
        b.free(g2)
        if sc is not x:
            b.free(sc)
        return out

    def forward(self, input_tensor, temb=None):
        b = eager_builder(input_tensor)
        x = to_nhwc(input_tensor, b.dtype)
        if temb is not None and (temb.dtype != b.dtype or not temb.is_contiguous()):
            temb = ops.convert(temb.contiguous(), b.dtype)
        return from_nhwc(self.emit(b, x, temb))


class Attention(nn.Module, _PackMixin):

    def __init__(self, query_dim, cross_attention_dim=None, heads=8, dim_head=64, bias=False, out_bias=True):
        super().__init__()
        inner = heads * dim_head
        self.heads, self.dim_head, self.inner = heads, dim_head, inner
        kv = query_dim if cross_attention_dim is None else cross_attention_dim
        self.to_q = Linear(query_dim, inner, bias=bias)
        self.to_k = Linear(kv, inner, bias=bias)
        self.to_v = Linear(kv, inner, bias=bias)
        self.to_out = nn.ModuleList([Linear(inner, query_dim, bias=out_bias), nn.Dropout(0.0)])

    def _packed_cat(self, dtype, mods: Sequence[Linear]):
        ws = [m.weight for m in mods]
        return self._cache(("cat", dtype, len(mods)), ws, lambda: ops.pack_weight(torch.cat([w.detach() for w in ws], 0), dtype))

    def _bias_cat(self, mods: Sequence[Linear]):
        if mods[0].bias is None:
            return None
        bs = [m.bias for m in mods]
        return self._cache(("bcat", len(mods)), bs, lambda: torch.cat([x.detach().float() for x in bs], 0).contiguous())

    def out_bias(self, extra: Optional[torch.Tensor] = None):
        bo = self.to_out[0].bias
        if extra is None:
            return self.to_out[0]._f32("bias")
        return self._cache(("bsum",), [bo, extra], lambda: (bo.detach().float() + extra.detach().float()).contiguous())

    def emit_self(self, b: Builder, xn, residual, seg, lens, extra_bias=None, name="attn", kv_lens=None):
        C = self.inner
        qkv = b.linear(xn, self._packed_cat(b.dtype, [self.to_q, self.to_k, self.to_v]),
                       self._bias_cat([self.to_q, self.to_k, self.to_v]), name=name + ".to_qkv")
        a = b.attention(qkv[:, :C], qkv[:, C:2 * C], qkv[:, 2 * C:], self.heads, self.dim_head, seg, lens, lens if kv_lens is None else kv_lens,
                        name=name + ".sdpa")
        b.free(qkv)
        out = b.linear(a, self.to_out[0].packed(b.dtype), self.out_bias(extra_bias), residual=residual, name=name + ".to_out")
        b.free(a)
        return out

    def emit_cross(self, b: Builder, xn, ctx, residual, seg, q_lens, kv_lens, name="attn"):
# ... 358 lines not shown
```

mv_ldm_amd/mvunet.py:

```python
from __future__ import annotations

import os

from dataclasses import dataclass, field
from typing import List, Optional, Sequence, Tuple

import torch
from torch import nn

from . import _lib as L
from . import ops
from .modules import (Attention, Builder, Conv2d, FeedForward, GroupNorm, LayerNorm, Linear, UNet2DConditionModel, _PackMixin,
                      _segments, eager_builder, weights_version)
from .runtime import from_nhwc, get_compute_dtype, require_gpu, to_nhwc


@dataclass
class SpatialTransformer3DCfg:
    name: str = "spatial_transformer_3d"
    num_heads: int = 8
    num_layers: int = 1
    d_dot: Optional[int] = None
    d_mlp: Optional[int] = None
    d_mlp_multiplier: Optional[int] = None
# ... 242 lines not shown
            with b.scope(f"transformer.layers.{i}"):
                a = attn.fn
                n1 = attn.norm.emit(b, hs, name="attn.norm")
                qkv = a.to_qkv.emit(b, n1, name="attn.to_qkv")
                b.free(n1)
                o = b.attention(qkv[:, :a.inner], qkv[:, a.inner:2 * a.inner], qkv[:, 2 * a.inner:], a.heads, a.dim_head,
                                _segments(b, lens), lens, lens, name="attn.sdpa")
                b.free(qkv)
                if isinstance(a.to_out, nn.Identity):
                    raise NotImplementedError("heads == 1 with dim_head == dim (no output projection)")
                h1 = a.to_out[0].emit(b, o, residual=hs, name="attn.to_out")
                b.free(o)
                if not first:
                    b.free(hs)
                n2 = ff.norm.emit(b, h1, name="ff.norm")
                g = ff.fn.net[0].emit(b, n2, epilogue=L.EPI_GELU, name="ff.net.0+gelu")
                b.free(n2)
                hs = ff.fn.net[3].emit(b, g, residual=h1, name="ff.net.3")
                b.free(g)
                b.free(h1)
                first = False
        return hs.view(n, h, w, c)

    def forward(self, features):
        bsz, v, c, h, w = features.shape
        b = eager_builder(features)
        y = self.emit(b, to_nhwc(features.reshape(bsz * v, c, h, w), b.dtype), [v] * bsz)
        return from_nhwc(y).reshape(bsz, v, c, h, w)


def get_attn_blocks(cfg, unet_blocks) -> nn.ModuleList:
    if cfg.name == "standard":
        return nn.ModuleList([StandardTransformer(cfg=cfg, d_in=block.resnets[-1].out_channels) for block in unet_blocks])
    if cfg.name == "spatial_transformer_3d":
        return nn.ModuleList([SpatialTransformer3D(cfg=cfg, d_in=block.resnets[-1].out_channels) for block in unet_blocks])
    raise NotImplementedError(f"multi_view_attention '{cfg.name}': the reference's get_attn_blocks knows 'standard' and "
                              "'spatial_transformer_3d' (src/model/denoiser/attention.py:12,21)")


class Denoiser(nn.Module):

    def __init__(self, cfg):
        super().__init__()
        self.cfg = cfg


class _PrefixDone(Exception):

    def __init__(self, skips):
        super().__init__()
        self.skips = skips


class MultiViewUNet(Denoiser, _PackMixin):
    def __init__(self, cfg: MultiViewUNetCfg, in_channels: int, out_channels: int):
        super().__init__(cfg)
        self.use_ray_encoding = cfg.use_ray_encoding
        self.pretrained_from = cfg.pretrained_from
        a = cfg.autoencoder
        if self.pretrained_from is None:
            self.unet = UNet2DConditionModel(
                in_channels=in_channels, out_channels=out_channels, down_block_types=a.down_block_types,
                mid_block_type=a.mid_block_type, up_block_types=a.up_block_types,
                only_cross_attention=a.only_cross_attention, block_out_channels=a.block_out_channels,
                cross_attention_dim=list(a.block_out_channels))
        else:
            self.unet = UNet2DConditionModel.from_pretrained(self.pretrained_from, subfolder="unet",
                                                             config_overrides=getattr(cfg, "pretrained_overrides", None),
                                                             state_dict=getattr(cfg, "pretrained_state_dict", None),
                                                             allow_random_init=getattr(cfg, "allow_random_init", False))
            c0 = self.unet.config.block_out_channels[0]
            self.unet.conv_in = Conv2d(in_channels, c0, kernel_size=3, padding=1)
            self.unet.conv_out = Conv2d(c0, out_channels, kernel_size=3, padding=1)
        if cfg.encoder_conditioning:
            self.cross_attn_blocks_encoder = get_attn_blocks(cfg.multi_view_attention, self.unet.down_blocks)
        if cfg.mid_conditioning:
            self.cross_attn_blocks_mid = get_attn_blocks(cfg.multi_view_attention, [self.unet.mid_block])
        if cfg.decoder_conditioning:
            self.cross_attn_blocks_decoder = get_attn_blocks(cfg.multi_view_attention, self.unet.up_blocks)
        self.in_channels, self.out_channels = in_channels, out_channels
        self._plans = {}

    def _resnets_in_order(self) -> List:
        u = self.unet
        rs = [r for blk in u.down_blocks for r in blk.resnets] + list(u.mid_block.resnets)
        return rs + [r for blk in u.up_blocks for r in blk.resnets]

    def _temb_proj_all(self, b: Builder, emb_act):
        rs = self._resnets_in_order()
        ws = [r.time_emb_proj.weight for r in rs]
        bs = [r.time_emb_proj.bias for r in rs]
        pw = self._cache(("tproj", b.dtype), ws, lambda: ops.pack_weight(torch.cat([w.detach() for w in ws], 0), b.dtype))
        bias = self._cache(("tprojb",), bs, lambda: torch.cat([x.detach().float() for x in bs], 0).contiguous())
        allp = b.linear(emb_act, pw, bias, out_dtype=torch.float32, name="time_emb_proj[all]")
        out, off = {}, 0
        for r in rs:
            out[id(r)] = allp[:, off:off + r.out_channels]
            off += r.out_channels
        return out

    def _zero_ctx_ok(self, cond_state) -> bool:
        return cond_state is None

    def emit(self, b: Builder, x_in, timesteps, groups: Sequence[int], out: Optional[torch.Tensor] = None,
             dup: Optional[tuple] = None, prefix_only: bool = False, tail: Optional[tuple] = None):
        u = self.unet
        n_img = x_in.shape[0]
        assert n_img == sum(groups)
        if dup is not None and (os.environ.get("MVLDM_CFG_SHARE", "1") == "0" or dup[0] >= n_img):
            dup = None
        const = None
        if dup is not None and len(dup) == 4:
            const = (dup[2], dup[3]) if os.environ.get("MVLDM_CFG_SHARE", "1") != "1a" else None
        n_src = n_img if dup is None else int(dup[0])
        shared = dup is not None
        lo, hi = (n_src, n_img) if const is not None else (0, n_src)
        with b.scope("time"):
            t_emb = u.time_proj.emit(b, timesteps, dtype=b.dtype)
            emb_act = u.time_embedding.emit(b, t_emb, silu_out=True)
            b.free(t_emb)
            tproj = self._temb_proj_all(b, emb_act)
            b.free(emb_act)

        def dest(shape_of):
            if not shared:
                return {}, None
            full = b.empty(n_img, *shape_of, dtype=b.dtype)
            return {"out": full[lo:hi]}, full

        def resnet(r, name, h, skip=None, **kw):
            with b.scope(name):
                tp_ = tproj[id(r)]
                return r.emit(b, h, None, x2=skip, temb_proj=tp_[lo:hi] if shared else tp_, **kw)

        def sd_attn(attn, name, h, **kw):
            with b.scope(name):
                return attn.emit(b, h, None, zero_ctx=True, **kw)

        fulls = {}

        def fill(full, i, name):
            if const is None:
                b.gather_rows(full, full[n_src:], src_index=dup[1], name=name)
            else:
                b.gather_rows(full[n_src:], full, dst_index=dup[1], name=name)
                b.gather_rows(const[1][i], full, dst_index=const[0], name=name + ".const")

        def expand(h):
            nonlocal shared
            if prefix_only:
                raise _PrefixDone(list(skips))
            if not shared:
                return h
            shared = False
            with b.scope("cfg_share"):
                for i, t in enumerate(skips):
                    full = fulls[id(t)]
                    fill(full, i, f"skip{i}")
                    skips[i] = full
                assert id(h) in fulls and any(fulls[id(h)] is t for t in skips), "the running activation at a multi-view block is a skip"
                return fulls[id(h)]

        def mv(blocks, idx, name, h, **kw):
            was_shared = shared
            h = expand(h)
            if (was_shared and isinstance(blocks[idx], SpatialTransformer3D) and len(groups) % 2 == 0
                    and os.environ.get("MVLDM_CFG_SHARE_ATTN", "1") != "0"):
                unc_img = torch.arange(n_src, n_img, dtype=torch.int32, device=b.device)
                b.keep.append(unc_img)
                kw = dict(kw, pair=(n_src, dup[1], unc_img))
            with b.scope(name):
                return blocks[idx].emit(b, h, groups, **kw)

        with b.scope("conv_in"):
            kw, full = dest((x_in.shape[1], x_in.shape[2], u.conv_in.out_channels))
            h = u.conv_in.emit(b, x_in[lo:hi] if shared else x_in, name="conv", **kw)
            if full is not None:
                fulls[id(h)] = full
        skips = [h]
        try:
            if tail is not None and os.environ.get("MVLDM_TAIL_DROP", "1") == "0":
                tail = None
            return self._emit_body(b, u, h, skips, fulls, dest, resnet, sd_attn, mv, expand, out, groups, tail)
        except _PrefixDone as done:
            return done.skips

    def _emit_body(self, b, u, h, skips, fulls, dest, resnet, sd_attn, mv, expand, out, groups, tail=None):
        live_mv = None
        compact = False
        n_img_full = sum(groups)
        for lvl, blk in enumerate(u.down_blocks):
            has_attn = getattr(blk, "has_cross_attention", False)
            for i, r in enumerate(blk.resnets):
                kw, full = ({}, None) if has_attn else dest((h.shape[1], h.shape[2], r.conv2.out_channels))
                nh = resnet(r, f"down{lvl}.resnets.{i}", h, **kw)
                if live_mv is not None:
                    b.free(live_mv)
                    live_mv = None
                h = nh
                if has_attn:
                    kw, full = dest(tuple(h.shape[1:]))
                    h2 = sd_attn(blk.attentions[i], f"down{lvl}.attentions.{i}", h, **kw)
                    b.free(h)
                    h = h2
                if full is not None:
                    fulls[id(h)] = full
                skips.append(h)
            if h.shape[1] <= 32 and h.shape[2] <= 32 and self.cfg.encoder_conditioning:
                h = mv(self.cross_attn_blocks_encoder, lvl, f"mv_encoder.{lvl}", h)
                live_mv = h
            if blk.downsamplers is not None:
                for d in blk.downsamplers:
                    with b.scope(f"down{lvl}.downsample"):
                        kw, full = dest(((h.shape[1] + 1) // 2, (h.shape[2] + 1) // 2, d.conv.out_channels))
                        nh = d.emit(b, h, **kw)
                        if full is not None:
                            fulls[id(nh)] = full
                    if live_mv is not None:
                        b.free(live_mv)
                        live_mv = None
                    h = nh
                skips.append(h)

        mid = u.mid_block
        h = expand(h)
        nh = resnet(mid.resnets[0], "mid.resnets.0", h)
        if live_mv is not None:
            b.free(live_mv)
            live_mv = None
        h = nh
        for i, (attn, r) in enumerate(zip(mid.attentions, mid.resnets[1:])):
            h2 = sd_attn(attn, f"mid.attentions.{i}", h)
            b.free(h)
            h3 = resnet(r, f"mid.resnets.{i + 1}", h2)
            b.free(h2)
            h = h3
        if self.cfg.mid_conditioning:
            h2 = mv(self.cross_attn_blocks_mid, 0, "mv_mid", h)
            b.free(h)
            h = h2

        for lvl, blk in enumerate(u.up_blocks):
            has_attn = getattr(blk, "has_cross_attention", False) and self.pretrained_from is None
            for i, r in enumerate(blk.resnets):
                skip = skips.pop()
                nh = resnet(r, f"up{lvl}.resnets.{i}", h, skip)
                b.free(h)
                b.free(skip)
                h = nh
                if has_attn:
                    h2 = sd_attn(blk.attentions[i], f"up{lvl}.attentions.{i}", h)
                    b.free(h)
                    h = h2
            if h.shape[1] <= 32 and h.shape[2] <= 32 and self.cfg.decoder_conditioning:
                drop_here = (tail is not None and lvl == len(u.up_blocks) - 1 and blk.upsamplers is None
                             and isinstance(self.cross_attn_blocks_decoder[lvl], SpatialTransformer3D))
                h2 = mv(self.cross_attn_blocks_decoder, lvl, f"mv_decoder.{lvl}", h, **({"keep": tail} if drop_here else {}))
                b.free(h)
                h = h2
                compact = drop_here
            if blk.upsamplers is not None:
                for up in blk.upsamplers:
                    with b.scope(f"up{lvl}.upsample"):
                        h2 = up.emit(b, h)
                    b.free(h)
                    h = h2
        with b.scope("out"):
            g = u.conv_norm_out.emit(b, h, silu=True, name="conv_norm_out+silu")
            b.free(h)
            if compact:
                eps_c = u.conv_out.emit(b, g, out_dtype=torch.float32, name="conv_out")
                eps = out if out is not None else b.empty(n_img_full, *eps_c.shape[1:], dtype=torch.float32)
                b.gather_rows(eps_c, eps, dst_index=tail[0], name="eps.scatter")
                b.free(eps_c)
            else:
                eps = u.conv_out.emit(b, g, out_dtype=torch.float32, out=out, name="conv_out")
            b.free(g)
        return eps

    def compile(self, b_scenes: int, views: int, h: int, w: int, dtype=None, graph: bool = True):
        dtype = dtype or get_compute_dtype()
        dev = next(self.parameters()).device
        key = (b_scenes, views, h, w, dtype, str(dev), graph)
        st = self._plans.get(key)
        if st is not None and st["weights_version"] == self.weights_version():
            return st
        n = b_scenes * views
        bld = Builder(dev, dtype, record=True)
        c_pad = (self.in_channels + ops.epc(dtype) - 1) // ops.epc(dtype) * ops.epc(dtype)
        lat = torch.zeros(n, self.in_channels, h, w, dtype=torch.float32, device=dev)
        ts = torch.zeros(n, dtype=torch.int64, device=dev)
        x_in = torch.zeros(n, h, w, c_pad, dtype=dtype, device=dev)
        out = torch.zeros(n, self.out_channels, h, w, dtype=torch.float32, device=dev)
        bld.nchw_to_nhwc(lat, x_in)
        eps = self.emit(bld, x_in, ts, [views] * b_scenes)
        bld.nhwc_to_nchw(eps, out)
        plan = bld.finalize()
        if graph:
            plan.capture()
        st = dict(plan=plan, lat=lat, ts=ts, out=out, graph=graph, weights_version=self.weights_version())
        self._plans[key] = st
# ... 77 lines not shown
```

mv_ldm_amd/ops.py:

```python
from __future__ import annotations

import ctypes as C
import os
from dataclasses import dataclass
from typing import Optional, Sequence

import math

import torch

from . import _lib as L

_DT = {torch.float32: L.F32, torch.bfloat16: L.BF16, torch.float16: L.F16}


def dt(t) -> int:
    return _DT[t if isinstance(t, torch.dtype) else t.dtype]


def epc(dtype: torch.dtype) -> int:
    return 4 if dtype == torch.float32 else 8


def stream() -> int:
# ... 90 lines not shown


def pack_job(w: torch.Tensor, pw: PackedWeight, *, transpose: bool = False, c_off: int = 0) -> "L.PackJob":
    assert w.is_cuda and w.dtype == torch.float32 and w.is_contiguous()
    j = L.PackJob()
    j.src, j.dst = w.data_ptr(), pw.data.data_ptr()
    j.n_out, j.c_in, j.ksize = w.shape[0], w.shape[1], pw.ksize
    j.c_pad, j.n_pad, j.k_pad, j.geglu, j.k_order = pw.c_pad, pw.n_pad, pw.k_pad, int(pw.geglu), pw.k_order
    j.transpose, j.c_off, j.n_rows = int(transpose), c_off, (pw.n_out if transpose else w.shape[0])
    L.check(L.load().mvldm_pack_job_prepare(C.byref(j), dt(pw.data.dtype)))
    return j


class PackBatch:

    def __init__(self, jobs: Sequence["L.PackJob"], dtype: torch.dtype, device):
        self.n, self.dtype = len(jobs), dtype
        arr = (L.PackJob * max(len(jobs), 1))()
        b0 = 0
        for i, j in enumerate(jobs):
            C.memmove(C.byref(arr[i]), C.byref(j), C.sizeof(L.PackJob))
            arr[i].block0 = b0
            b0 += j.blocks
        self.total_blocks = b0
        raw = torch.frombuffer(bytearray(bytes(arr)), dtype=torch.uint8).clone()
        self.table = raw.to(device)
        self.block_job = None
        if jobs:
            self.block_job = torch.repeat_interleave(torch.arange(len(jobs), dtype=torch.int32), torch.tensor([j.blocks for j in jobs])).to(device)
            assert self.block_job.numel() == b0

    def run(self):
        L.check(L.load().mvldm_pack_weight_batch(self.table.data_ptr(), self.n, None if self.block_job is None else self.block_job.data_ptr(),
                                                 self.total_blocks, dt(self.dtype), stream()))


def conv_out_hw(h: int, w: int, ksize: int, stride: int, pad: int, upsample) -> tuple:
    if int(upsample) >= 2:
        return h, w
    hs, ws = (2 * h, 2 * w) if upsample else (h, w)
    if ksize == 3 and stride == 2 and pad == 0:
        return (hs + 1 - 3) // 2 + 1, (ws + 1 - 3) // 2 + 1
    return (hs + 2 * pad - ksize) // stride + 1, (ws + 2 * pad - ksize) // stride + 1


def use_skinny(d, pw: PackedWeight) -> torch.Tensor:
    t = pw.skinny()
    d.weight, d.k_order = ptr(t), 2
    return t


def igemm_desc(src0, src1, pw: PackedWeight, dst, *, n_img, h_in, w_in, h_out, w_out, stride=1, pad=None, upsample=False,
               bias=None, row_bias=None, residual=None, epilogue=L.EPI_NONE, out_scale=1.0, ws=None, splitk=0,
               tile=0, into=None) -> L.IgemmDesc:
    d = L.IgemmDesc() if into is None else into
    c0 = src0.shape[-1]
    c1 = 0 if src1 is None else src1.shape[-1]
    assert c0 + c1 == pw.c_pad, f"weight packed for {pw.c_pad} channels, sources give {c0}+{c1}"
    assert not pw.k_order or c0 % block_k(src0.dtype) == 0, "weight packed block-major but the source split is unaligned"
    d.src0, d.src1, d.weight = ptr(src0), ptr(src1), ptr(pw.data)
    d.bias, d.row_bias, d.residual, d.dst = ptr(bias), ptr(row_bias), ptr(residual), ptr(dst)
    d.c0, d.c1 = c0, c1
    d.n_img, d.h_in, d.w_in, d.h_out, d.w_out = n_img, h_in, w_in, h_out, w_out
    d.ksize, d.stride, d.upsample = pw.ksize, stride, int(upsample)
    d.pad = (pw.ksize // 2) if pad is None else pad
    d.n_out, d.n_pad, d.k_pad = pw.n_out, pw.n_pad, pw.k_pad
    d.row_bias_ld = 0 if row_bias is None else row_bias.stride(0)
    d.epilogue, d.act_dtype, d.dst_dtype = epilogue, dt(src0), dt(dst)
    d.splitk, d.tile, d.out_scale = splitk, tile, out_scale
    n_dst = pw.n_out // 2 if epilogue == L.EPI_GEGLU else pw.n_out
    d.dst_ld = 0 if dst.shape[-1] == n_dst else dst.shape[-1]
    d.k_order = pw.k_order
    if (tile & 63) == 15:
        use_skinny(d, pw)
    if ws is not None:
        d.workspace, d.workspace_bytes = ws.data_ptr(), ws.numel() * ws.element_size()
    else:
        d.workspace, d.workspace_bytes = None, 0
        if splitk == 0:
            d.splitk = 1
    return d


def conv2d(x: torch.Tensor, pw: PackedWeight, bias=None, *, x2=None, stride=1, pad=None, upsample=False, row_bias=None,
           residual=None, epilogue=L.EPI_NONE, out_dtype=None, out_scale=1.0, splitk=0, tile=0, out=None, dst=None) -> torch.Tensor:
    assert x.is_cuda and x.is_contiguous() and (x2 is None or x2.is_contiguous())
    n, h, w, _ = x.shape
    pad = (pw.ksize // 2) if pad is None else pad
    ho, wo = conv_out_hw(h, w, pw.ksize, stride, pad, upsample)
    n_dst = pw.n_out // 2 if epilogue == L.EPI_GEGLU else pw.n_out
    if dst is not None:
        up = 2 if int(upsample) >= 2 else 1
        assert out is None and dst.is_contiguous() and dst.dtype == (out_dtype or x.dtype) and dst.shape[-1] > n_dst
        assert dst.numel() == n * up * ho * up * wo * dst.shape[-1]
        out = dst
    elif out is None:
        out = torch.empty(n, ho, wo, n_dst, dtype=out_dtype or x.dtype, device=x.device)
    else:
        assert out.is_contiguous() and out.numel() == n * ho * wo * n_dst and out.dtype == (out_dtype or x.dtype)
        out = out.view(n, ho, wo, n_dst)
    scratch = None
    if splitk != 1:
        scratch = workspace(min(16 * n * ho * wo * pw.n_pad * 4, 256 << 20), x.device)
    d = igemm_desc(x, x2, pw, out, n_img=n, h_in=h, w_in=w, h_out=ho, w_out=wo, stride=stride, pad=pad,
                   upsample=upsample, bias=bias, row_bias=row_bias, residual=residual, epilogue=epilogue,
                   out_scale=out_scale, ws=scratch, splitk=splitk, tile=tile)
    L.check(L.load().mvldm_igemm_fwd(C.byref(d), stream()))
    return out


def upsample_phase_weights(w: torch.Tensor) -> list:
    assert w.ndim == 4 and w.shape[2:] == (3, 3)
    w = w.detach().to(torch.float32)
    rows = {0: (w[:, :, 0], w[:, :, 1] + w[:, :, 2]), 1: (w[:, :, 0] + w[:, :, 1], w[:, :, 2])}
    out = []
    for py in (0, 1):
        for px in (0, 1):
            taps = []
            for r in rows[py]:
                cols = (r[:, :, 0], r[:, :, 1] + r[:, :, 2]) if px == 0 else (r[:, :, 0] + r[:, :, 1], r[:, :, 2])
                taps.append(torch.stack(cols, dim=-1))
            out.append(torch.stack(taps, dim=-2).contiguous())
    return out


def conv2d_upsample_phases(x: torch.Tensor, pws, bias=None, tile=0, splitk=0) -> torch.Tensor:
    n, h, w, _ = x.shape
    out = torch.empty(n, 2 * h, 2 * w, pws[0].n_out, dtype=x.dtype, device=x.device)
    scratch = workspace(min(16 * n * h * w * pws[0].n_pad * 4, 256 << 20), x.device)
    for phase, pw in enumerate(pws):
        d = igemm_desc(x, None, pw, out, n_img=n, h_in=h, w_in=w, h_out=h, w_out=w, stride=1, pad=0, upsample=2 + phase,
                       bias=bias, splitk=splitk, tile=tile, ws=scratch)
        L.check(L.load().mvldm_igemm_fwd(C.byref(d), stream()))
    return out


def linear(x: torch.Tensor, pw: PackedWeight, bias=None, *, residual=None, epilogue=L.EPI_NONE, out_dtype=None,
           splitk=0, tile=0, out=None, dst=None) -> torch.Tensor:
    rows, c = x.shape
    y = conv2d(x.view(rows, 1, 1, c), pw, bias, residual=None if residual is None else residual.view(rows, 1, 1, -1),
               epilogue=epilogue, out_dtype=out_dtype, splitk=splitk, tile=tile, out=out, dst=None if dst is None else dst.view(rows, 1, 1, -1))
    return y.view(rows, -1)


def groupnorm(x: torch.Tensor, gamma, beta, groups: int, eps: float, silu: bool, x2=None, stats_out=None, out=None) -> torch.Tensor:
    assert x.is_cuda and x.is_contiguous() and (x2 is None or x2.is_contiguous())
    n, c0 = x.shape[0], x.shape[-1]
    c1 = 0 if x2 is None else x2.shape[-1]
    hw = math.prod(x.shape[1:-1])
    if out is None:
        y = torch.empty(*x.shape[:-1], c0 + c1, dtype=x.dtype, device=x.device)
    else:
        assert out.is_contiguous() and out.dtype == x.dtype and out.numel() == n * hw * (c0 + c1)
        y = out.view(*x.shape[:-1], c0 + c1)
    ws = workspace(max(n, 1) * L.GN_MAX_CHUNKS * groups * 2 * 8, x.device, "gn")
    L.check(L.load().mvldm_groupnorm_fwd(x.data_ptr(), ptr(x2), y.data_ptr(), gamma.data_ptr(), beta.data_ptr(), n, hw, c0, c1,
                                         groups, eps, int(silu), dt(x), ws.data_ptr(), ptr(stats_out), stream()))
    return y

# ... 584 lines not shown
```

mv_ldm_amd/pipeline.py:

```python
from __future__ import annotations

import os

from dataclasses import dataclass
from typing import Optional

import torch

from . import ops
from .mvunet import MultiViewUNet
from .plan import Builder
from .runtime import compute_dtype, get_compute_dtype
from .scheduler import DDIMScheduler
from .vae import AutoencoderKL

VAE_SCALE = 0.18215


def sample_image_grid(shape, device="cpu", dtype=torch.float32):
    h, w = shape
    ys = ((torch.arange(h, device=device) + 0.5) / h).to(dtype)
    xs = ((torch.arange(w, device=device) + 0.5) / w).to(dtype)
    gx, gy = torch.meshgrid(xs, ys, indexing="xy")
    ii, jj = torch.meshgrid(torch.arange(h, device=device), torch.arange(w, device=device), indexing="ij")
# ... 133 lines not shown
            return self.scheduler.step(pred_c[:, v_c:].contiguous(), ts, x_t, generator=step_generator, variance_noise=step_noise).prev_sample
        return self.scheduler.step(pred_c[:, v_c:].contiguous(), ts, x_t).prev_sample

    def _ancestral(self) -> bool:
        from .scheduler import DDPMScheduler
        return isinstance(self.scheduler, DDPMScheduler)

    def _cfg_ddim(self, pred_c, pred_u, x_t, ts):
        dev = x_t.device
        coef = self.scheduler.step_coefficients(int(ts)).reshape(1, 4).to(dev)
        zero = torch.zeros(1, dtype=torch.int32, device=dev)
        eps = torch.stack([pred_c.float().reshape(-1), pred_u.float().reshape(-1)]).view(2, 1, -1, 1).contiguous()
        out = ops.ddim_cfg_step(eps, x_t.float().contiguous().view(1, 1, -1, 1), zero, torch.ones(1, dtype=torch.int32, device=dev),
                                self.cfg.cfg_scale, coef, zero, None, clip_range=self.scheduler.clip_range)
        return out.view(x_t.shape)

    def _compile(self, b: int, v_c: int, v_t: int, hl: int, wl: int, dtype, n_steps: int):
        sch = self.scheduler
        key = (b, v_c, v_t, hl, wl, dtype, n_steps, self.cfg.use_cfg, self.cfg.cfg_scale, str(self.device),
               tuple(int(t) for t in sch.timesteps), sch.clip_range, tuple(sorted(self.rays.kernel_args().items())))
        st = self._plans.get(key)
        if st is not None and st["weights_version"] == self.denoiser.weights_version():
            return st
        dev, den = self.device, self.denoiser
        lc = den.out_channels
        use_cfg = self.cfg.use_cfg
        v = v_c + v_t
        n_cond, n_unc = b * v, (b * v_t if use_cfg else 0)
        n_img = n_cond + n_unc
        e = ops.epc(dtype)
        c_pad = (den.in_channels + e - 1) // e * e
        unet_in = torch.zeros(n_img, hl, wl, c_pad, dtype=dtype, device=dev)
        x_state = torch.zeros(b * v_t, hl, wl, lc, dtype=torch.float32, device=dev)
        eps = torch.zeros(n_img, hl, wl, lc, dtype=torch.float32, device=dev)
        timesteps = torch.zeros(n_img, dtype=torch.int64, device=dev)
        cond_img = torch.tensor([s * v + v_c + j for s in range(b) for j in range(v_t)], dtype=torch.int32, device=dev)
        unc_img = (torch.tensor([n_cond + s * v_t + j for s in range(b) for j in range(v_t)], dtype=torch.int32, device=dev)
                   if use_cfg else None)
        tgt_rows = cond_img if not use_cfg else torch.cat([cond_img, unc_img])
        t_table = sch.timesteps.to(dev, torch.int64).contiguous()
        coef = sch.coefficient_table().to(dev)
        step_ptr = torch.zeros(1, dtype=torch.int32, device=dev)
        groups = [v] * b + ([v_t] * b if use_cfg else [])
        ctx_rows = torch.tensor([s * v + j for s in range(b) for j in range(v_c)], dtype=torch.int32, device=dev)
        dup, const_plan = None, None
        if use_cfg and v_c > 0 and os.environ.get("MVLDM_CFG_SHARE", "1") != "0":
            dup = (n_cond, cond_img)
            if os.environ.get("MVLDM_CFG_SHARE", "1") != "1a":
                cb = Builder(dev, dtype, record=True)
                x_ctx = torch.zeros(b * v_c, hl, wl, c_pad, dtype=dtype, device=dev)
                t_ctx = torch.zeros(b * v_c, dtype=torch.int64, device=dev)
                cb.gather_rows(unet_in, x_ctx, src_index=ctx_rows, name="context rows")
                with cb.scope("unet_ctx"):
                    const_skips = den.emit(cb, x_ctx, t_ctx, [1] * (b * v_c), prefix_only=True)
                cb.keep.extend([x_ctx, t_ctx, *const_skips])
                const_plan = cb.finalize()
                dup = (n_cond, cond_img, ctx_rows, const_skips)
        bld = Builder(dev, dtype, record=True)
        with bld.scope("unet"):
            tail = (tgt_rows, [v_c] * b + ([0] * b if use_cfg else [])) if v_c > 0 else None
            den.emit(bld, unet_in, timesteps, groups, out=eps, dup=dup, tail=tail)
        bld.ddim_step(eps, x_state, x_state, cond_img, unc_img, self.cfg.cfg_scale, coef, step_ptr, unet_in,
                      clip_range=sch.clip_range)
        bld.ddim_advance(step_ptr, t_table, timesteps, tgt_rows)
        plan = bld.finalize()
        plan.capture()
        ctx_lat = torch.zeros(b * v_c, lc, hl, wl, dtype=torch.float32, device=dev)
        x_T = torch.zeros(b * v_t, lc, hl, wl, dtype=torch.float32, device=dev)
        ones = torch.ones(b * v_t, 1, hl, wl, dtype=torch.float32, device=dev)
        extr = torch.zeros(n_img, 4, 4, dtype=torch.float32, device=dev)
        intr = torch.zeros(n_img, 3, 3, dtype=torch.float32, device=dev)
        minus_one = torch.full((1,), -1, dtype=torch.int32, device=dev)
        ld = Builder(dev, dtype, record=True)
        ld.memcpy(step_ptr, minus_one, name="step_ptr=-1")
        ld.ddim_advance(step_ptr, t_table, timesteps, tgt_rows, name="step 0 / timesteps[targets] = t_0")
        ld.nchw_to_nhwc(ctx_lat, unet_in, 0, img_map=ctx_rows, name="context latents")
        for rows in ((cond_img, unc_img) if use_cfg else (cond_img,)):
            ld.nchw_to_nhwc(x_T, unet_in, 0, img_map=rows, name="x_T")
            ld.nchw_to_nhwc(ones, unet_in, lc, img_map=rows, name="target mask")
        ld.ray_encode(extr, intr, hl, wl, unet_in, lc + 1, name="ray grid", **self.rays.kernel_args())
        ld.nchw_to_nhwc(x_T, x_state, 0, name="x_T -> fp32 state")
        loader = ld.finalize(autotune=False)
        st = dict(plan=plan, loader=loader, const_plan=const_plan, unet_in=unet_in, x_state=x_state, eps=eps, timesteps=timesteps, cond_img=cond_img,
                  unc_img=unc_img, tgt_rows=tgt_rows, t_table=t_table, step_ptr=step_ptr, n_cond=n_cond,
                  ctx_lat=ctx_lat, x_T=x_T, extr=extr, intr=intr, weights_version=den.weights_version())
        self._plans[key] = st
        return st

    def load_inputs(self, st, ctx_latents, x_T, ctx_cams, tgt_cams):
        b, v_t = x_T.shape[:2]
        st["ctx_lat"].copy_(ctx_latents.reshape(st["ctx_lat"].shape))
        st["x_T"].copy_(x_T.reshape(st["x_T"].shape))
        n_cond = st["n_cond"]
        for buf, ci, ti, k in ((st["extr"], ctx_cams[0], tgt_cams[0], 4), (st["intr"], ctx_cams[1], tgt_cams[1], 3)):
            allc = torch.cat([ci.reshape(b, -1, k, k), ti.reshape(b, -1, k, k)], dim=1).to(torch.float32)
            buf[:n_cond].copy_(allc.reshape(n_cond, k, k))
            if st["unc_img"] is not None:
                buf[n_cond:].copy_(ti.reshape(b * v_t, k, k))
        st["loader"].run()
        if st.get("const_plan") is not None:
            st["const_plan"].run()

    def _scaled_noise(self, x_T):
        sigma = self.scheduler.init_noise_sigma
        return x_T if sigma == 1.0 else x_T * sigma

    def _read_state(self, st, b, v_t):
# ... 108 lines not shown
```

mv_ldm_amd/plan.py:

```python
from __future__ import annotations

import ctypes as C
import json
import os
import sys
from dataclasses import dataclass
from typing import List, Optional

import torch

from . import _lib as L
from .ops import PackedWeight, conv_out_hw, dt, igemm_desc, ptr, use_skinny


def _PIN_TILE() -> int:
    v = os.environ.get("MVLDM_IGEMM_TILE")
    return int(v) if v else 0


@dataclass
class OpMeta:
    name: str
    kind: int
    flops: float = 0.0
# ... 73 lines not shown
        op.kind = kind
        self._emit(op, name)

    def splitk_ws(self) -> torch.Tensor:
        if self._lane:
            ws = self._lane_ws.get(("splitk", self._lane))
            if ws is None:
                ws = torch.empty(min(self._ws_bytes, 64 << 20), dtype=torch.uint8, device=self.device)
                self._lane_ws[("splitk", self._lane)] = ws
                self.keep.append(ws)
            return ws
        if self._ws is None:
            self._ws = torch.empty(self._ws_bytes, dtype=torch.uint8, device=self.device)
            self.keep.append(self._ws)
        return self._ws

    def gn_ws(self, n_img: int, groups: int) -> torch.Tensor:
        need = n_img * L.GN_MAX_CHUNKS * groups * 16
        if self._lane:
            ws = self._lane_ws.get(("gn", self._lane))
            if ws is None or ws.numel() < need:
                ws = torch.empty(max(need, 1 << 16), dtype=torch.uint8, device=self.device)
                self._lane_ws[("gn", self._lane)] = ws
                self.keep.append(ws)
            return ws
        if self._gn_ws is None or self._gn_ws.numel() < need:
            self._gn_ws = torch.empty(max(need, 1 << 16), dtype=torch.uint8, device=self.device)
            self.keep.append(self._gn_ws)
        return self._gn_ws

    class _Scope:
        def __init__(self, b, name):
            self.b, self.name = b, name

        def __enter__(self):
            self.b._scope.append(self.name)

        def __exit__(self, *a):
            self.b._scope.pop()

    def scope(self, name: str):
        return Builder._Scope(self, name)

    def _emit(self, op: L.Op, name: str, flops=0.0, nbytes=0.0, refs=()):
        if self.record:
            op.tag = len(self.ops)
            self.ops.append(op)
            self.meta.append(OpMeta("/".join(self._scope + [name]), op.kind, flops, nbytes))
            self.keep.extend(r for r in refs if r is not None)
        else:
            L.check(L.load().mvldm_op_run(C.byref(op), torch.cuda.current_stream().cuda_stream))

    def conv(self, x, pw: PackedWeight, bias=None, *, x2=None, stride=1, pad=None, upsample=False, row_bias=None,
             residual=None, epilogue=L.EPI_NONE, out_dtype=None, out_scale=1.0, out=None, name="conv", splitk=0, tile=0):
        n, h, w, c0 = x.shape
        c1 = 0 if x2 is None else x2.shape[-1]
        pad = (pw.ksize // 2) if pad is None else pad
        ho, wo = conv_out_hw(h, w, pw.ksize, stride, pad, upsample)
        n_dst = pw.n_out // 2 if epilogue == L.EPI_GEGLU else pw.n_out
        if out is None:
            out = self.empty(n, ho, wo, n_dst, dtype=out_dtype or x.dtype)
        ws = self.splitk_ws() if splitk != 1 else None
        if tile == 0 and _PIN_TILE() and x.dtype != torch.float32 and pw.k_order == 1:
            tile, splitk = _PIN_TILE(), 1
        m = n * ho * wo
        k_real = pw.ksize * pw.ksize * (c0 + c1)
        es = x.element_size()
        nbytes = (pw.n_out * k_real + n * h * w * (c0 + c1)) * es + m * n_dst * out.element_size() \
            + (m * n_dst * es if residual is not None else 0)
        self._igemm(x, x2, pw, bias, row_bias, residual, out, ws, name, 2.0 * m * pw.n_out * k_real, nbytes, h_out=ho, w_out=wo,
                    stride=stride, pad=pad, upsample=upsample, epilogue=epilogue, out_scale=out_scale, splitk=splitk, tile=tile)
        return out

    def _igemm(self, x, x2, pw, bias, row_bias, residual, out, ws, name, flops, nbytes, *, h_out, w_out, tile=0, **desc):
        n, h, w, c0 = x.shape
        c1 = 0 if x2 is None else x2.shape[-1]
        op = L.Op()
        op.kind = L.OP_IGEMM
        d = igemm_desc(x, x2, pw, out, n_img=n, h_in=h, w_in=w, h_out=h_out, w_out=w_out, bias=bias, row_bias=row_bias,
                       residual=residual, ws=ws, tile=tile, into=op.u.igemm, **desc)
        m = n * h_out * w_out
        can_sk = tile == 0 and self.skinny and skinny_candidate(pw, m, c0, c1, d.upsample, x.dtype) \
            and x.is_cuda and L.load().mvldm_igemm_skinny_config(C.byref(d)) > 0
        if can_sk and skinny_rule(m, pw.n_pad):
            tile = d.tile = 15
            use_skinny(d, pw)
        elif can_sk and self.record:
            self._skinny_pw[len(self.ops)] = pw
        if self.record:
            own = self.__dict__.get("_own_ptrs", ())
            self.__dict__.setdefault("_tune_srcs", {})[len(self.ops)] = tuple(t if (t is not None and t.data_ptr() in own) else None
                                                                              for t in (x, x2))
        self._emit(op, name, flops, nbytes, (x, x2, pw.data, pw._skinny if (tile & 63) == 15 else None, bias, row_bias, residual, out))

    def small_launch(self, rows: int, n_out: int) -> bool:
        limit = int(os.environ.get("MVLDM_PAR_ROWS", "0"))
        return self.record and rows * max(n_out, 1) <= limit * 640 and limit > 0

    def conv_upsample_phases(self, x, pws, bias=None, name="upsample"):
        n, h, w, c0 = x.shape
        out = self.empty(n, 2 * h, 2 * w, pws[0].n_out, dtype=x.dtype)
        lanes = self.parallel() if self.small_launch(n * h * w, pws[0].n_out) else None
        if lanes is not None:
            lanes.__enter__()
        for phase, pw in enumerate(pws):
            if lanes is not None:
                lanes.lane()
            self._phase_conv(x, pw, bias, out, phase, name)
        if lanes is not None:
            lanes.__exit__(None, None, None)
        return out

    def _phase_conv(self, x, pw, bias, out, phase, name, tile=0, splitk=0):
        n, h, w, c0 = x.shape
        ws = self.splitk_ws()
        assert pw.ksize == 2 and pw.k_order == 1 and c0 == pw.c_pad
        m = n * h * w
        es = x.element_size()
        nbytes = (pw.n_out * 4 * c0 + (m * c0 if phase == 0 else 0)) * es + m * pw.n_out * es
        self._igemm(x, None, pw, bias, None, None, out, ws, f"{name}.p{phase}", 2.0 * m * pw.n_out * 4 * c0, nbytes, h_out=h, w_out=w,
                    stride=1, pad=0, upsample=2 + phase, splitk=splitk, tile=tile)

    def linear(self, x, pw: PackedWeight, bias=None, *, residual=None, epilogue=L.EPI_NONE, out_dtype=None, out=None,
               name="linear", row_bias=None):
        rows, c = x.shape
        y = self.conv(x.view(rows, 1, 1, c), pw, bias, residual=None if residual is None else residual.view(rows, 1, 1, -1),
                      epilogue=epilogue, out_dtype=out_dtype, out=None if out is None else out.view(rows, 1, 1, -1),
                      name=name, row_bias=row_bias)
        return y.view(rows, -1)

    def groupnorm(self, x, gamma, beta, groups, eps, silu, x2=None, name="groupnorm", stats_out=None):
        n, c0 = x.shape[0], x.shape[-1]
        c1 = 0 if x2 is None else x2.shape[-1]
        hw = x.numel() // (n * c0)
        y = self.empty(*x.shape[:-1], c0 + c1, dtype=x.dtype)
        op = L.Op()
        op.kind = L.OP_GROUPNORM
        g = op.u.groupnorm
        g.x, g.x1, g.y, g.gamma, g.beta = ptr(x), ptr(x2), ptr(y), ptr(gamma), ptr(beta)
        g.stats_ws = self.gn_ws(n, groups).data_ptr()
        g.n_img, g.hw, g.c0, g.c1, g.groups, g.silu, g.dtype, g.eps = n, hw, c0, c1, groups, int(silu), dt(x), eps
        g.stats_out = ptr(stats_out)
        passes = L.load().mvldm_groupnorm_passes(n, hw, c0 + c1, groups, dt(x))
        self._emit(op, name, 0.0, float(passes) * y.numel() * y.element_size(), (x, x2, y, gamma, beta, stats_out))
        return y

# ... 156 lines not shown
_SPLIT_CACHE = {}
_VALIDATED = set()
_TUNE_TILES = tuple(int(t) for t in os.environ["MVLDM_TUNE_TILES"].split(",")) if os.environ.get("MVLDM_TUNE_TILES") else (0, 1, 2, 3, 4, 5, 6, 7, 8, 9, 10, 11, 12, 13, 14)


def tune_cache_state() -> dict:
    return {"version": 2, "igemm": {json.dumps(list(k)): (int(v) if isinstance(v, int) else list(v)) for k, v in _TUNE_CACHE.items()},
            "wgrad": {json.dumps(list(k)): int(v) for k, v in _WGRAD_CACHE.items()},
            "split": {json.dumps(list(k)): int(v) for k, v in _SPLIT_CACHE.items()}}


def set_tune_cache_state(state: dict, replace: bool = False) -> None:
    if replace:
        _TUNE_CACHE.clear()
        _WGRAD_CACHE.clear()
        _SPLIT_CACHE.clear()
    for name, cache in (("igemm", _TUNE_CACHE), ("wgrad", _WGRAD_CACHE), ("split", _SPLIT_CACHE)):
        for k, v in (state.get(name) or {}).items():
            cache[tuple(json.loads(k))] = int(v) if isinstance(v, int) else list(v)


def save_tune_cache(path: Optional[str] = None) -> Optional[str]:
    path = path or os.environ.get("MVLDM_TUNE_CACHE")
    if not path:
        return None
    tmp = f"{path}.{os.getpid()}.tmp"
    with open(tmp, "w") as f:
        json.dump(tune_cache_state(), f, indent=0, sort_keys=True)
    os.replace(tmp, path)
    return path


def load_tune_cache(path: Optional[str] = None) -> int:
    path = path or os.environ.get("MVLDM_TUNE_CACHE")
    if not path or not os.path.exists(path):
        return 0
    with open(path) as f:
        set_tune_cache_state(json.load(f))
    return len(_TUNE_CACHE) + len(_WGRAD_CACHE) + len(_SPLIT_CACHE)


def broadcast_tune_cache(dist, src: int = 0, device=None) -> None:
    box = [tune_cache_state() if dist.get_rank() == src else None]
    dist.broadcast_object_list(box, src=src, device=device)
    set_tune_cache_state(box[0], replace=True)


load_tune_cache()


def _igemm_signature(d) -> tuple:
    return (d.n_img, d.h_in, d.w_in, d.h_out, d.w_out, d.c0, d.c1, d.ksize, d.stride, d.pad, d.upsample, d.n_out, d.n_pad,
            d.k_pad, d.epilogue, d.act_dtype, d.dst_dtype, d.k_order, d.dst_ld, bool(d.residual), bool(d.row_bias),
            bool(d.bias), d.splitk, d.workspace_bytes)


_SMALL_ROWS = int(os.environ.get("MVLDM_TUNE_SMALL_ROWS", "64"))
_SPLITS = (0, 1, 2, 4, 8, 16, 32)
_MID_ROWS = int(os.environ.get("MVLDM_TUNE_MID_ROWS", "40000"))
_MID_SPLITS = (0, 1, 2, 3, 4, 6, 8)
_SMALL_TILES = tuple(int(t) for t in os.environ.get("MVLDM_TUNE_SMALL_TILES", "0,1,2,3,4,5").split(","))


_SKINNY = os.environ.get("MVLDM_SKINNY", "1") != "0"
_SKINNY_ROWS = int(os.environ.get("MVLDM_SKINNY_ROWS", "2304"))
_SKINNY_CFGS = tuple(int(c) for c in os.environ.get("MVLDM_SKINNY_CFGS", "0,1,2,5,6,7,8,9,10,12,13,18,19,20,38,39,40,41,42,43,44,46").split(","))


def skinny_rule(rows: int, n_pad: int) -> bool:
    if os.environ.get("MVLDM_AUTOTUNE", "1") != "0" or os.environ.get("MVLDM_SKINNY_RULE", "1") == "0":
        return False
    return rows <= 160 or (rows <= 1152 and n_pad <= 1280)


def skinny_candidate(pw: PackedWeight, rows: int, c0: int, c1: int, upsample, dtype) -> bool:
    return (_SKINNY and dtype != torch.float32 and rows <= _SKINNY_ROWS and not (upsample is True or upsample == 1) and pw.can_skinny()
            and c0 % 64 == 0 and c1 % 64 == 0)


def _unpack_choice(v):
    return (int(v), None) if isinstance(v, int) else (int(v[0]), None if v[1] is None else int(v[1]))


_TUNE_COLD = int(os.environ.get("MVLDM_TUNE_COLD", "9216"))
_THRASH = []
_THRASH_FILLS = [0]


def _thrash(device=None):
    if not _THRASH or (device is not None and _THRASH[0].device != torch.device(device)):
        _THRASH[:] = [torch.empty(640 << 20, dtype=torch.uint8, device=torch.cuda.current_device() if device is None else device)]
    return _THRASH[0]


def autotune_igemm(ops, min_rows: int = 2048, iters: int = 4, srcs=None, skinny=None, keep=None) -> int:
    lib = L.load()
    stream = torch.cuda.current_stream().cuda_stream
    e0, e1 = torch.cuda.Event(enable_timing=True), torch.cuda.Event(enable_timing=True)
    timed = 0
    tune_dev = next((t.device for pair in (srcs or {}).values() for t in pair if t is not None), None)
    if srcs:
        seen, gen = set(), None
        for pair in srcs.values():
            for t in pair:
                if t is not None and t.is_floating_point() and t.data_ptr() not in seen:
                    seen.add(t.data_ptr())
                    if gen is None:
# ... 83 lines not shown
            d.splitk = sk
        if (tile & 63) == 15:
            t = use_skinny(d, sk_pw)
            sk_pw._skinny_pinned = True
            if keep is not None:
                keep.append(t)
        elif sk_pw is not None:
            sk_pw.drop_skinny()
    if timed:
        save_tune_cache()
        _THRASH.clear()
    return timed


_BATCH_SPLIT = os.environ.get("MVLDM_BATCH_SPLIT", "1") != "0"
_SPLIT_MIN_ROWS = int(os.environ.get("MVLDM_BATCH_SPLIT_MIN_ROWS", "16384"))


def _split_candidates(d) -> list:
    rpi = d.h_out * d.w_out
    rows = d.n_img * rpi
    out = []
    for bn in (320, 256):
        n_tiles = -(-d.n_pad // bn)
        m_tiles = -(-rows // 256)
        if m_tiles * n_tiles <= 256 or (m_tiles * n_tiles) % 256 == 0 or (m_tiles * n_tiles) % 256 > 216:
            continue
        for m1 in range(m_tiles - 1, 0, -1):
            if (m1 * n_tiles) % 256 == 0 and (m1 * 256) % rpi == 0:
                n1 = m1 * 256 // rpi
                frac = 1.0 - n1 / d.n_img
                if 0.03 <= frac <= 0.45 and n1 not in out:
                    out.append(n1)
                break
    return out


def _image_range(op, i0: int, n: int):
    q = L.Op()
    C.memmove(C.byref(q), C.byref(op), C.sizeof(L.Op))
    d = q.u.igemm
    es = 4 if d.act_dtype == L.F32 else 2
    ds = 4 if d.dst_dtype == L.F32 else 2
    n_dst = d.n_out // 2 if d.epilogue == L.EPI_GEGLU else d.n_out
    px_in, px_out = d.h_in * d.w_in, d.h_out * d.w_out

    def off(p, nbytes):
        return (p + nbytes) if p else p
    d.src0 = off(d.src0, i0 * px_in * d.c0 * es)
    d.src1 = off(d.src1, i0 * px_in * d.c1 * es)
    d.dst = off(d.dst, i0 * px_out * (d.dst_ld or n_dst) * ds)
    d.residual = off(d.residual, i0 * px_out * n_dst * es)
    d.row_bias = off(d.row_bias, i0 * d.row_bias_ld * 4)
    d.n_img = n
    d.tile, d.splitk = 0, 0
    return q


def _time_ops(ops, iters: int) -> float:
    lib = L.load()
    stream = torch.cuda.current_stream().cuda_stream
    e0, e1 = torch.cuda.Event(enable_timing=True), torch.cuda.Event(enable_timing=True)
    for o in ops:
        L.check(lib.mvldm_op_run(C.byref(o), stream))
    e0.record()
    for _ in range(iters):
        for o in ops:
            lib.mvldm_op_run(C.byref(o), stream)
    e1.record()
    e1.synchronize()
    return e0.elapsed_time(e1) / iters


def autosplit_igemm(ops, meta, skinny=None, keep=None, iters: int = 6):
    new_ops, new_meta, decided = [], [], 0
    for idx, (op, m) in enumerate(zip(ops, meta)):
        d = op.u.igemm if op.kind == L.OP_IGEMM else None
        rows = d.n_img * d.h_out * d.w_out if d is not None else 0
        ok = (d is not None and rows >= _SPLIT_MIN_ROWS and d.act_dtype != L.F32 and d.k_order == 1 and d.stride == 1 and not d.upsample
              and (d.tile & 63) != 15 and not _PIN_TILE() and bool(d.workspace) and idx not in (skinny or {}))
        n1 = 0
        if ok:
            key = _igemm_signature(d)[:-2] + (d.workspace_bytes,)
            if key in _SPLIT_CACHE:
                n1 = _SPLIT_CACHE[key]
            else:
                best_t, t_whole = None, None
                for cand in _split_candidates(d):
                    parts = [_image_range(op, 0, cand), _image_range(op, cand, d.n_img - cand)]
                    try:
                        autotune_igemm(parts, iters=4)
                        if t_whole is None:
                            t_whole = _time_ops([op], iters)
                        t = _time_ops(parts, iters)
                    except L.MvldmError:
                        continue
                    if os.environ.get("MVLDM_BATCH_SPLIT_LOG"):
                        print(f"[batch split] {m.name}: {d.n_img} images x {d.h_out}x{d.w_out}, N {d.n_out}, K {d.k_pad}: whole {t_whole * 1e3:.1f} us (tile {d.tile & 63}, "
                              f"splitk {d.splitk}); {cand} + {d.n_img - cand}: {t * 1e3:.1f} us (tiles {parts[0].u.igemm.tile & 63} / {parts[1].u.igemm.tile & 63}, "
                              f"splitk {parts[1].u.igemm.splitk})", file=sys.stderr, flush=True)
                    if t < 0.97 * t_whole and (best_t is None or t < best_t):
                        best_t, n1 = t, cand
                _SPLIT_CACHE[key] = n1
                decided += 1
        if n1:
            parts = [_image_range(op, 0, n1), _image_range(op, n1, d.n_img - n1)]
# ... 112 lines not shown
```

Before: 49.69.

## Add per-image fp32 addend to igemm epilogue to share context-view prefix work

Adds an addend/addend_map pair to the implicit-GEMM descriptor so the epilogue can add a precomputed fp32 tensor, indexed per image through a map, before activation. The UNet prefix on the constant context views is emitted with partial_rows, and skip tensors are shared through _SkipShare objects, so constant context contributions are computed once and folded in instead of being recomputed every step. Split-K, GEGLU, phase convs and some tiles are rejected when an addend is present, which can force less efficient tile or split choices. It also adds an extra fp32 read per output element.

Measured after the change: 49.30. About the same (-0.8%).

```diff
diff --git a/include/mvldm.h b/include/mvldm.h
--- a/include/mvldm.h
+++ b/include/mvldm.h
@@ -46,6 +46,8 @@
     int32_t dst_ld;
     float out_scale;
     size_t workspace_bytes;
+    const float* addend;
+    const int32_t* addend_map;
 } mvldm_igemm_desc;
 int mvldm_igemm_fwd(const mvldm_igemm_desc* d, mvldm_stream_t stream);
 size_t mvldm_igemm_workspace_bytes(const mvldm_igemm_desc* d);
diff --git a/mv_ldm_amd/_lib.py b/mv_ldm_amd/_lib.py
--- a/mv_ldm_amd/_lib.py
+++ b/mv_ldm_amd/_lib.py
@@ -30,7 +30,8 @@
                 ("ksize", i32), ("stride", i32), ("pad", i32), ("upsample", i32),
                 ("n_out", i32), ("n_pad", i32), ("k_pad", i32),
                 ("row_bias_ld", i32), ("epilogue", i32), ("act_dtype", i32), ("dst_dtype", i32),
-                ("splitk", i32), ("tile", i32), ("k_order", i32), ("dst_ld", i32), ("out_scale", f32), ("workspace_bytes", sz)]
+                ("splitk", i32), ("tile", i32), ("k_order", i32), ("dst_ld", i32), ("out_scale", f32), ("workspace_bytes", sz),
+                ("addend", vp), ("addend_map", vp)]
 
 
 class _GroupNorm(C.Structure):
diff --git a/mv_ldm_amd/csrc/igemm.hip b/mv_ldm_amd/csrc/igemm.hip
--- a/mv_ldm_amd/csrc/igemm.hip
+++ b/mv_ldm_amd/csrc/igemm.hip
@@ -133,7 +133,7 @@
 
 static thread_local int t_force_sync = 0;
 
-static int launch_igemm(const IgemmParams& p, int tile, int act_dtype, hipStream_t s) {
+static int launch_igemm(const IgemmParamsA& p, int tile, int act_dtype, hipStream_t s) {
     if (tile >= 1 && tile <= 5) return igemm_launch_small(p, tile, act_dtype, s);
     if (tile >= 6 && tile <= 8) return igemm_launch_large(p, tile, act_dtype, s);
     if (tile == 9 || tile == 10 || tile == 18) return igemm_launch_xl(p, tile, act_dtype, s);
@@ -171,7 +171,7 @@
     splitk = std::max(1, std::min(splitk, k_tiles));
 }
 
-static int fill_params(const mvldm_igemm_desc& d, IgemmParams& p, int& tile) {
+static int fill_params(const mvldm_igemm_desc& d, IgemmParamsA& p, int& tile) {
     const int epc = d.act_dtype == MVLDM_F32 ? 4 : 8;
     const int bk = d.act_dtype == MVLDM_F32 ? 32 : 64;
     MVLDM_REQUIRE(d.src0 && d.weight && d.dst, "igemm: null pointer");
@@ -191,6 +191,10 @@
         MVLDM_REQUIRE(d.n_out % 64 == 0 && !d.row_bias, "igemm: GEGLU needs n_out %% 64 == 0");
     p.src0 = d.src0; p.src1 = d.src1; p.weight = d.weight; p.bias = d.bias; p.row_bias = d.row_bias;
     p.residual = d.residual; p.dst = d.dst; p.ws = d.workspace;
+    p.addend = d.addend; p.addend_map = d.addend_map;
+    p.add_vec = d.addend && ((uintptr_t)d.addend % 16 == 0) && d.n_out % 4 == 0;
+    if (d.addend && (d.epilogue == MVLDM_EPI_GEGLU || phase))
+        return set_error(MVLDM_ERR_UNSUPPORTED, "igemm: the GEGLU epilogue and the 2x2 phase convs do not take an addend");
     p.c0 = d.c0; p.c1 = d.c1; p.ctot = d.c0 + d.c1;
     p.n_img = d.n_img; p.h_in = d.h_in; p.w_in = d.w_in; p.h_out = d.h_out; p.w_out = d.w_out;
     p.hw_out = d.h_out * d.w_out;
@@ -212,6 +216,11 @@
     const int force_px = (d.tile >> 8) & 15;
     int splitk = d.splitk;
     MVLDM_REQUIRE(((tile >= 0 && tile <= kNumTiles) || tile == 17 || deep_tile(tile)) && splitk >= 0, "igemm: tile/splitk");
+    if (d.addend) {
+        if (splitk > 1) return set_error(MVLDM_ERR_UNSUPPORTED, "igemm: split-K does not take an addend");
+        if (tile == 11 || tile == 17) return set_error(MVLDM_ERR_UNSUPPORTED, "igemm: tile %d does not take an addend", tile);
+        splitk = 1;
+    }
     choose_config(d, p.M, p.k_tiles, tile, splitk, d.workspace_bytes);
     if (splitk > 1)
         MVLDM_REQUIRE(d.workspace && (size_t)splitk * p.M * d.n_pad * sizeof(float) <= d.workspace_bytes,
@@ -308,10 +317,13 @@
 int linear_rs_run(const mvldm_igemm_desc& d, hipStream_t s);
 
 int igemm_run(const mvldm_igemm_desc& d, hipStream_t s) {
-    IgemmParams p;
+    IgemmParamsA p;
     int tile = 0;
     if (d.n_img == 0 || d.h_out == 0 || d.w_out == 0) return MVLDM_OK;
     const int req = d.tile & 63;
+    MVLDM_REQUIRE((d.addend == nullptr) == (d.addend_map == nullptr), "igemm: addend and addend_map come together");
+    if (d.addend && (req == 15 || req == 12 || req == 13 || req == 14 || req == 19))
+        return set_error(MVLDM_ERR_UNSUPPORTED, "igemm: tile %d does not take an addend", req);
     if (req == 15) return skinny_run(d, s);
     if (req == 12 || req == 13 || req == 14 || req == 19) {
         MVLDM_REQUIRE(d.src0 && d.weight && d.dst, "igemm: null pointer");
@@ -330,13 +342,13 @@
                 if (!p.dst_f32 && p.n_dst % 8 == 0 && p.dst_ld % 8 == 0 && ((uintptr_t)p.ws % 16) == 0 &&
                     (!p.residual || ((uintptr_t)p.residual % 16) == 0) && ((uintptr_t)p.dst % 16) == 0) {
                     const size_t chunks = (size_t)p.M * (p.n_dst / 8);
-                    hipLaunchKernelGGL(igemm_splitk_reduce_vec<T>, dim3((unsigned)std::min<size_t>((chunks + 255) / 256, 4096)), dim3(256), 0, s, p);
+                    hipLaunchKernelGGL(igemm_splitk_reduce_vec<T>, dim3((unsigned)std::min<size_t>((chunks + 255) / 256, 4096)), dim3(256), 0, s, static_cast<const IgemmParams&>(p));
                     return check_launch();
                 }
             }
             const size_t total = (size_t)p.M * p.n_dst;
             const int blocks = (int)std::min<size_t>((total + 255) / 256, 4096);
-            hipLaunchKernelGGL(igemm_splitk_reduce<T>, dim3(blocks), dim3(256), 0, s, p);
+            hipLaunchKernelGGL(igemm_splitk_reduce<T>, dim3(blocks), dim3(256), 0, s, static_cast<const IgemmParams&>(p));
             return check_launch();
         }
         return (int)MVLDM_OK;
diff --git a/mv_ldm_amd/csrc/igemm_bl.h b/mv_ldm_amd/csrc/igemm_bl.h
--- a/mv_ldm_amd/csrc/igemm_bl.h
+++ b/mv_ldm_amd/csrc/igemm_bl.h
@@ -4,7 +4,7 @@
 namespace mvldm {
 
 template <typename T, int BM, int BN, int WM, int WN>
-__global__ __launch_bounds__(WM* WN * 64) void igemm_kernel(const IgemmParams p) {
+__global__ __launch_bounds__(WM* WN * 64) void igemm_kernel(const IgemmParamsA p) {
     using M_ = Mma<T>;
     constexpr int NT = WM * WN * 64;
     constexpr int EPC = Elt<T>::EPC;
@@ -143,7 +143,7 @@
 };
 
 template <typename T, int BM, int BN, int NW, int KS, bool DUAL, int A_IT, int B_IT, int STAGES, bool UPS, int t, int LO = 0, int HI = 1 << 20>
-__device__ __forceinline__ void bl_issue(const IgemmParams& p, char* stage_base, int wave, int cb,
+__device__ __forceinline__ void bl_issue(const IgemmParamsA& p, char* stage_base, int wave, int cb,
                                          const BlAddr<KS * KS, A_IT, DUAL, UPS>& ad, const unsigned (&vb)[B_IT]) {
     constexpr int BK = 64, TAPS = KS * KS;
     const int lead = (!UPS && KS > 1) ? p.w_in + 1 : 0;
@@ -208,7 +208,7 @@
 }
 
 template <typename T, int BM, int BN, int WM, int WN, int KS, bool DUAL, int STAGES, bool UPS>
-__global__ __launch_bounds__(WM* WN * 64) void igemm_bl_kernel(const IgemmParams p) {
+__global__ __launch_bounds__(WM* WN * 64) void igemm_bl_kernel(const IgemmParamsA p) {
     using M_ = Mma<T>;
     static_assert(sizeof(T) == 2, "16-bit activation types only");
     constexpr int NW = WM * WN, TAPS = KS * KS;
@@ -439,7 +439,7 @@
     }
 }
 
-template <typename T, int BM, int BN, int WM, int WN> static int launch_sync(const IgemmParams& p, hipStream_t s) {
+template <typename T, int BM, int BN, int WM, int WN> static int launch_sync(const IgemmParamsA& p, hipStream_t s) {
     static std::atomic<uint64_t> done{0};
     constexpr int ring = 2 * (BM + BN) * Mma<T>::PITCH, park = WM * WN * 32 * (park_blocks(BN / WN / 32) * 32 + 4) * 4;
     return launch_kernel(igemm_kernel<T, BM, BN, WM, WN>, done, (sizeof(T) == 2 && park > ring) ? park : ring,
@@ -447,14 +447,14 @@
 }
 
 template <typename T, int BM, int BN, int WM, int WN, int KS, bool DUAL, int STAGES, bool UPS>
-static int launch_bl_s(const IgemmParams& p, hipStream_t s) {
+static int launch_bl_s(const IgemmParamsA& p, hipStream_t s) {
     static std::atomic<uint64_t> done{0};
     constexpr int ring = STAGES * (BM + BN) * 128, park = WM * WN * 32 * (park_blocks(BN / WN / 32) * 32 + 4) * 4;
     return launch_kernel(igemm_bl_kernel<T, BM, BN, WM, WN, KS, DUAL, STAGES, UPS>, done, ring > park ? ring : park,
                          8 * p.sub_m * p.sub_n * p.splitk, WM * WN * 64, p, s);
 }
 template <typename T, int BM, int BN, int WM, int WN, int KS, bool DUAL, int DEPTH = 0>
-static int launch_bl(const IgemmParams& p, hipStream_t s) {
+static int launch_bl(const IgemmParamsA& p, hipStream_t s) {
     constexpr int STAGES = DEPTH ? DEPTH : ((WM * WN == 8 && 3 * (BM + BN) * 128 <= 160 * 1024) ? 3 : 2);
     if (p.upsample) {
         if constexpr (KS == 3 && !DUAL && ((BM == 128 && BN == 64) || (BM == 256 && BN == 128)))
@@ -464,14 +464,14 @@
     }
     return launch_bl_s<T, BM, BN, WM, WN, KS, DUAL, STAGES, false>(p, s);
 }
-template <typename T, int BM, int BN, int WM, int WN, int DEPTH> static int launch_bl_deep(const IgemmParams& p, hipStream_t s) {
+template <typename T, int BM, int BN, int WM, int WN, int DEPTH> static int launch_bl_deep(const IgemmParamsA& p, hipStream_t s) {
     const bool dual = p.c1 > 0;
     if (p.ksize == 3) return dual ? launch_bl<T, BM, BN, WM, WN, 3, true, DEPTH>(p, s) : launch_bl<T, BM, BN, WM, WN, 3, false, DEPTH>(p, s);
     if (p.ksize == 1) return dual ? launch_bl<T, BM, BN, WM, WN, 1, true, DEPTH>(p, s) : launch_bl<T, BM, BN, WM, WN, 1, false, DEPTH>(p, s);
     return set_error(MVLDM_ERR_ARG, "igemm: the deep-ring tiles take 1x1 and 3x3 convs");
 }
 
-template <typename T, int BM, int BN, int WM, int WN> static int launch_bl_any(const IgemmParams& p, hipStream_t s) {
+template <typename T, int BM, int BN, int WM, int WN> static int launch_bl_any(const IgemmParamsA& p, hipStream_t s) {
     const bool dual = p.c1 > 0;
     if (p.ksize == 2) {
         if constexpr ((BM == 128 && BN == 64) || (BM == 256 && BN == 128) || (BM == 256 && BN == 320))
@@ -489,7 +489,7 @@
     return dual ? launch_bl<T, BM, BN, WM, WN, 1, true>(p, s) : launch_bl<T, BM, BN, WM, WN, 1, false>(p, s);
 }
 
-template <typename T, int BM, int BN, int WM, int WN> static int launch_tile(const IgemmParams& p, hipStream_t s) {
+template <typename T, int BM, int BN, int WM, int WN> static int launch_tile(const IgemmParamsA& p, hipStream_t s) {
     if constexpr (sizeof(T) == 2) {
         if (p.use_bl) return launch_bl_any<T, BM, BN, WM, WN>(p, s);
     }
diff --git a/mv_ldm_amd/csrc/igemm_common.h b/mv_ldm_amd/csrc/igemm_common.h
--- a/mv_ldm_amd/csrc/igemm_common.h
+++ b/mv_ldm_amd/csrc/igemm_common.h
@@ -1,5 +1,6 @@
 #pragma once
 #include <algorithm>
+#include <type_traits>
 
 #include "common.h"
 
@@ -29,6 +30,13 @@
     int nt_store;
 };
 
+struct IgemmParamsA : IgemmParams {
+    const float* addend;
+    const int* addend_map;
+    int add_vec;
+};
+template <typename P> constexpr bool has_addend = std::is_same<P, IgemmParamsA>::value;
+
 template <typename T> struct Mma;
 
 template <typename T16> struct Mma16 : Mfma16<T16> {
@@ -107,8 +115,8 @@
     return tm < p.tiles_m && tn < p.tiles_n;
 }
 
-template <typename T, int BM, int BN, int WM, int WN>
-__device__ __forceinline__ void igemm_epilogue(const IgemmParams& p, f32x16 (&acc)[BM / WM / 32][BN / WN / 32], int tm, int tn,
+template <typename T, int BM, int BN, int WM, int WN, typename P>
+__device__ __forceinline__ void igemm_epilogue(const P& p, f32x16 (&acc)[BM / WM / 32][BN / WN / 32], int tm, int tn,
                                                int split, int wm, int wn, int hi, int l31) {
     constexpr int TM = BM / WM / 32, TN = BN / WN / 32;
     const bool geglu = p.epilogue == MVLDM_EPI_GEGLU;
@@ -158,6 +166,12 @@
                     if (m >= p.M) continue;
                     float v = acc[i][j][r] + bv;
                     if (p.row_bias) v += p.row_bias[(size_t)(m / p.hw_out) * p.row_bias_ld + n];
+                    if constexpr (has_addend<P>) {
+                        if (p.addend) {
+                            const int img = m / p.hw_out;
+                            v += p.addend[((size_t)p.addend_map[img] * p.hw_out + (m - img * p.hw_out)) * p.n_out + n];
+                        }
+                    }
                     if (p.epilogue == MVLDM_EPI_SILU) v = silu_f(v);
                     else if (p.epilogue == MVLDM_EPI_GELU) v = gelu_erf_fast(v);
                     epilogue_store<T>(p, m, n, v);
@@ -171,8 +185,29 @@
 
 enum { EPI_PLAIN = 0, EPI_ACT_SILU = 1, EPI_PAIR_GEGLU = 2, EPI_PARTIAL = 3, EPI_ACT_GELU = 4 };
 
-template <typename T, int JN, int MODE, int PITCH>
-__device__ __forceinline__ void epi_rows(const IgemmParams& p, const float* st, int m0, int pcol0, int split, int lane) {
+template <typename P>
+__device__ __forceinline__ void add_row(const P& p, int m, int n0, int img0, size_t base0, f32x4& x0, f32x4& x1) {
+    if constexpr (has_addend<P>) {
+        if (m >= p.M) return;
+        size_t arow;
+        if (img0 >= 0) arow = base0 + (size_t)(m - img0 * p.hw_out);
+        else {
+            const int img = m / p.hw_out;
+            arow = (size_t)p.addend_map[img] * p.hw_out + (size_t)(m - img * p.hw_out);
+        }
+        const float* ap = p.addend + arow * p.n_out + n0;
+        if (p.add_vec) {
+            x0 = *reinterpret_cast<const f32x4*>(ap);
+            x1 = *reinterpret_cast<const f32x4*>(ap + 4);
+        } else {
+#pragma unroll
+            for (int e = 0; e < 4; ++e) { x0[e] = ap[e]; x1[e] = ap[4 + e]; }
+        }
+    }
+}
+
+template <typename T, int JN, int MODE, int PITCH, bool AHEAD, typename P>
+__device__ __forceinline__ void epi_rows(const P& p, const float* st, int m0, int pcol0, int split, int lane) {
     constexpr bool PAIR = MODE == EPI_PAIR_GEGLU;
     constexpr int WC = PAIR ? JN * 16 : JN * 32;
     constexpr int CPR = WC / 8;
@@ -229,10 +264,32 @@
             for (int e = 0; e < 4; ++e) { rbv[e] = r0[e]; rbv[4 + e] = r1[e]; }
         }
     }
+    [[maybe_unused]] bool add_on = false;
+    [[maybe_unused]] f32x4 ad0 = {0.f, 0.f, 0.f, 0.f}, ad1 = {0.f, 0.f, 0.f, 0.f};
+    [[maybe_unused]] int add_img0 = -1;
+    [[maybe_unused]] size_t add_base0 = 0;
+    if constexpr (has_addend<P> && MODE != EPI_PARTIAL && MODE != EPI_PAIR_GEGLU) {
+        add_on = p.addend != nullptr;
+        if (add_on) {
+            const int img0 = m0 / p.hw_out;
+            if ((min(m0 + 31, p.M - 1) / p.hw_out) == img0) {
+                add_img0 = img0;
+                add_base0 = (size_t)p.addend_map[img0] * p.hw_out;
+            }
+            if constexpr (AHEAD) add_row<P>(p, m0 + row0, n0, add_img0, add_base0, ad0, ad1);
+        }
+    }
 #pragma unroll
     for (int it = 0; it < ITERS; ++it) {
         const int row = row0 + it * RSTEP;
         const int m = m0 + row;
+        if constexpr (has_addend<P> && MODE != EPI_PARTIAL && MODE != EPI_PAIR_GEGLU && !AHEAD) {
+            if (add_on) add_row<P>(p, m, n0, add_img0, add_base0, ad0, ad1);
+        }
+        [[maybe_unused]] const f32x4 ac0 = ad0, ac1 = ad1;
+        if constexpr (has_addend<P> && MODE != EPI_PARTIAL && MODE != EPI_PAIR_GEGLU && AHEAD) {
+            if (add_on && it + 1 < ITERS) add_row<P>(p, m + RSTEP, n0, add_img0, add_base0, ad0, ad1);
+        }
         if (m >= p.M) continue;
         const f32x4 a = *reinterpret_cast<const f32x4*>(st + row * PITCH + voff);
         const f32x4 b = *reinterpret_cast<const f32x4*>(st + row * PITCH + voff + 4);
@@ -265,6 +322,12 @@
                         for (int e = 0; e < 8; ++e) v[e] += rb[e];
                     }
                 }
+                if constexpr (has_addend<P>) {
+                    if (add_on) {
+#pragma unroll
+                        for (int e = 0; e < 4; ++e) { v[e] += ac0[e]; v[4 + e] += ac1[e]; }
+                    }
+                }
                 if constexpr (MODE == EPI_ACT_SILU) {
 #pragma unroll
                     for (int e = 0; e < 8; ++e) v[e] = silu_f(v[e]);
@@ -306,18 +369,18 @@
         for (int r = 0; r < 16; ++r) st[((r & 3) + 8 * (r >> 2) + 4 * hi) * PITCH + j * 32 + l31] = acc[I][J0 + j][r];
 }
 
-template <typename T, int JN, int PITCH>
-__device__ __forceinline__ void epi_group_rows(const IgemmParams& p, const float* st, int m0, int pcol0, int split, int mode, int lane) {
-    if (mode == EPI_PARTIAL) epi_rows<T, JN, EPI_PARTIAL, PITCH>(p, st, m0, pcol0, split, lane);
+template <typename T, int JN, int PITCH, bool AHEAD, typename P>
+__device__ __forceinline__ void epi_group_rows(const P& p, const float* st, int m0, int pcol0, int split, int mode, int lane) {
+    if (mode == EPI_PARTIAL) epi_rows<T, JN, EPI_PARTIAL, PITCH, AHEAD>(p, st, m0, pcol0, split, lane);
     else if (mode == EPI_PAIR_GEGLU) {
-        if constexpr (JN % 2 == 0) epi_rows<T, JN, EPI_PAIR_GEGLU, PITCH>(p, st, m0, pcol0, split, lane);
-    } else if (mode == EPI_ACT_SILU) epi_rows<T, JN, EPI_ACT_SILU, PITCH>(p, st, m0, pcol0, split, lane);
-    else if (mode == EPI_ACT_GELU) epi_rows<T, JN, EPI_ACT_GELU, PITCH>(p, st, m0, pcol0, split, lane);
-    else epi_rows<T, JN, EPI_PLAIN, PITCH>(p, st, m0, pcol0, split, lane);
-}
-
-template <typename T, int BM, int BN, int WM, int WN, int I>
-__device__ __forceinline__ void igemm_epilogue_rowblock(const IgemmParams& p, const f32x16 (&acc)[BM / WM / 32][BN / WN / 32], float* st, int tm, int tn,
+        if constexpr (JN % 2 == 0) epi_rows<T, JN, EPI_PAIR_GEGLU, PITCH, AHEAD>(p, st, m0, pcol0, split, lane);
+    } else if (mode == EPI_ACT_SILU) epi_rows<T, JN, EPI_ACT_SILU, PITCH, AHEAD>(p, st, m0, pcol0, split, lane);
+    else if (mode == EPI_ACT_GELU) epi_rows<T, JN, EPI_ACT_GELU, PITCH, AHEAD>(p, st, m0, pcol0, split, lane);
+    else epi_rows<T, JN, EPI_PLAIN, PITCH, AHEAD>(p, st, m0, pcol0, split, lane);
+}
+
+template <typename T, int BM, int BN, int WM, int WN, int I, typename P>
+__device__ __forceinline__ void igemm_epilogue_rowblock(const P& p, const f32x16 (&acc)[BM / WM / 32][BN / WN / 32], float* st, int tm, int tn,
                                                         int split, int wm, int wn, int mode, int lane) {
     constexpr int TM = BM / WM / 32, TN = BN / WN / 32;
     constexpr int WCOLS = BN / WN;
@@ -326,16 +389,17 @@
     const int m0 = tm * BM + wm * (BM / WM) + I * 32;
     const int pcol0 = tn * BN + wn * WCOLS;
     epi_park<TM, TN, I, 0, JG, PITCH>(acc, st, lane);
-    epi_group_rows<T, JG, PITCH>(p, st, m0, pcol0, split, mode, lane);
+    constexpr bool AHEAD = WM * WN == 8;
+    epi_group_rows<T, JG, PITCH, AHEAD>(p, st, m0, pcol0, split, mode, lane);
     if constexpr (TN > JG) {
         epi_park<TM, TN, I, JG, TN - JG, PITCH>(acc, st, lane);
-        epi_group_rows<T, TN - JG, PITCH>(p, st, m0, pcol0 + JG * 32, split, mode, lane);
+        epi_group_rows<T, TN - JG, PITCH, AHEAD>(p, st, m0, pcol0 + JG * 32, split, mode, lane);
     }
     if constexpr (I + 1 < TM) igemm_epilogue_rowblock<T, BM, BN, WM, WN, I + 1>(p, acc, st, tm, tn, split, wm, wn, mode, lane);
 }
 
-template <typename T, int BM, int BN, int WM, int WN>
-__device__ __forceinline__ void igemm_epilogue_staged(const IgemmParams& p, f32x16 (&acc)[BM / WM / 32][BN / WN / 32], int tm,
+template <typename T, int BM, int BN, int WM, int WN, typename P>
+__device__ __forceinline__ void igemm_epilogue_staged(const P& p, f32x16 (&acc)[BM / WM / 32][BN / WN / 32], int tm,
                                                       int tn, int split, int wm, int wn, int wave, int lane, char* smem) {
     constexpr int TN = BN / WN / 32;
     constexpr int JG = park_blocks(TN);
@@ -398,8 +462,8 @@
 constexpr int kNumTiles = 11;
 inline bool deep_tile(int tile) { return tile == 18; }
 
-template <typename KernT> inline int launch_kernel(KernT kern, std::atomic<uint64_t>& attr_done, int smem, int blocks, int threads,
-                                                   const IgemmParams& p, hipStream_t s) {
+template <typename KernT, typename P> inline int launch_kernel(KernT kern, std::atomic<uint64_t>& attr_done, int smem, int blocks, int threads,
+                                                               const P& p, hipStream_t s) {
     if (int rc0 = ensure_dyn_smem(reinterpret_cast<const void*>(kern), smem, attr_done)) return rc0;
     hipLaunchKernelGGL(kern, dim3(blocks), dim3(threads), smem, s, p);
     return check_launch();
@@ -415,9 +479,9 @@
 }
 template <typename F> inline int dispatch_16bit(int dtype, F&& f) { return dtype == MVLDM_BF16 ? f(bf16_t{}) : f(f16_t{}); }
 
-int igemm_launch_small(const IgemmParams& p, int tile, int act_dtype, hipStream_t s);
-int igemm_launch_large(const IgemmParams& p, int tile, int act_dtype, hipStream_t s);
-int igemm_launch_xl(const IgemmParams& p, int tile, int act_dtype, hipStream_t s);
+int igemm_launch_small(const IgemmParamsA& p, int tile, int act_dtype, hipStream_t s);
+int igemm_launch_large(const IgemmParamsA& p, int tile, int act_dtype, hipStream_t s);
+int igemm_launch_xl(const IgemmParamsA& p, int tile, int act_dtype, hipStream_t s);
 int igemm_launch_halo(const IgemmParams& p, int tile, int act_dtype, hipStream_t s);
 
 }
diff --git a/mv_ldm_amd/csrc/igemm_large.hip b/mv_ldm_amd/csrc/igemm_large.hip
--- a/mv_ldm_amd/csrc/igemm_large.hip
+++ b/mv_ldm_amd/csrc/igemm_large.hip
@@ -2,7 +2,7 @@
 
 namespace mvldm {
 
-int igemm_launch_large(const IgemmParams& p, int tile, int act_dtype, hipStream_t s) {
+int igemm_launch_large(const IgemmParamsA& p, int tile, int act_dtype, hipStream_t s) {
     if (int rc = require_bl(p, tile, act_dtype)) return rc;
     return dispatch_16bit(act_dtype, [&](auto t) {
         using T = decltype(t);
diff --git a/mv_ldm_amd/csrc/igemm_small.hip b/mv_ldm_amd/csrc/igemm_small.hip
--- a/mv_ldm_amd/csrc/igemm_small.hip
+++ b/mv_ldm_amd/csrc/igemm_small.hip
@@ -2,7 +2,7 @@
 
 namespace mvldm {
 
-int igemm_launch_small(const IgemmParams& p, int tile, int act_dtype, hipStream_t s) {
+int igemm_launch_small(const IgemmParamsA& p, int tile, int act_dtype, hipStream_t s) {
     return dispatch_dtype(act_dtype, [&](auto t) {
         using T = decltype(t);
         switch (tile) {
diff --git a/mv_ldm_amd/csrc/igemm_xl.hip b/mv_ldm_amd/csrc/igemm_xl.hip
--- a/mv_ldm_amd/csrc/igemm_xl.hip
+++ b/mv_ldm_amd/csrc/igemm_xl.hip
@@ -2,7 +2,7 @@
 
 namespace mvldm {
 
-int igemm_launch_xl(const IgemmParams& p, int tile, int act_dtype, hipStream_t s) {
+int igemm_launch_xl(const IgemmParamsA& p, int tile, int act_dtype, hipStream_t s) {
     if (tile == 18) {
         if (p.epilogue == MVLDM_EPI_GEGLU) return set_error(MVLDM_ERR_UNSUPPORTED, "igemm: tile 18 does not take the GEGLU epilogue");
         if (act_dtype == MVLDM_F32 || !p.use_bl || p.upsample)
diff --git a/mv_ldm_amd/csrc/skinny.hip b/mv_ldm_amd/csrc/skinny.hip
--- a/mv_ldm_amd/csrc/skinny.hip
+++ b/mv_ldm_amd/csrc/skinny.hip
@@ -692,7 +692,7 @@
 }
 
 bool skinny_applicable(const mvldm_igemm_desc& d) {
-    if (d.act_dtype == MVLDM_F32 || d.k_order != 2) return false;
+    if (d.act_dtype == MVLDM_F32 || d.k_order != 2 || d.addend) return false;
     if (!(d.ksize == 1 || d.ksize == 3 || (d.ksize == 2 && d.upsample >= 2)) || (d.upsample == 1)) return false;
     if (d.ksize != 2 && d.upsample != 0) return false;
     if (d.c0 % 64 || d.c1 % 64 || d.c0 <= 0 || (d.c1 == 0) != (d.src1 == nullptr)) return false;
diff --git a/mv_ldm_amd/modules.py b/mv_ldm_amd/modules.py
--- a/mv_ldm_amd/modules.py
+++ b/mv_ldm_amd/modules.py
@@ -178,14 +178,54 @@
         self.nonlinearity = nn.SiLU()
         self.conv_shortcut = Conv2d(in_channels, out_channels, 1) if in_channels != out_channels else None
 
-    def emit(self, b: Builder, x, temb=None, x2=None, temb_proj=None, out=None):
+    def skip_split(self, c_skip: int) -> Optional[int]:
+        c_h = self.in_channels - c_skip
+        gs = self.in_channels // self.norm1.num_groups
+        if self.conv_shortcut is None or c_h <= 0 or c_skip <= 0 or self.in_channels % self.norm1.num_groups:
+            return None
+        return c_h if c_h % gs == 0 and c_h % 64 == 0 and c_skip % 64 == 0 else None
+
+    def _half_pack(self, conv: "Conv2d", dtype, lo: int, hi: int) -> PackedWeight:
+        return conv._cache(("w_cols", dtype, lo, hi), [conv.weight], lambda: ops.pack_weight(conv.weight.detach()[:, lo:hi].contiguous(), dtype))
+
+    def emit_skip_partials(self, b: Builder, skip, c_h: int, p_out, s_out):
+        gs, c_in = self.in_channels // self.norm1.num_groups, self.in_channels
+        gamma, beta = self.norm1._f32("weight"), self.norm1._f32("bias")
+        n_s = b.groupnorm(skip, gamma[c_h:], beta[c_h:], (c_in - c_h) // gs, self.norm1.eps, True, name="norm1+silu.skip")
+        b.conv(n_s, self._half_pack(self.conv1, b.dtype, c_h, c_in), None, out=p_out, name="conv1.skip")
+        b.free(n_s)
+        b.conv(skip, self._half_pack(self.conv_shortcut, b.dtype, c_h, c_in), None, out=s_out, name="conv_shortcut.skip")
+
+    def emit(self, b: Builder, x, temb=None, x2=None, temb_proj=None, out=None, skip_share=None):
         if self.time_emb_proj is not None and temb_proj is None:
             ta = b.eltwise(temb, L.ELT_SILU, name="temb_silu")
             temb_proj = self.time_emb_proj.emit(b, ta, out_dtype=torch.float32, name="time_emb_proj")
             b.free(ta)
+        if skip_share is not None:
+            assert x2 is None and self.skip_split(self.in_channels - x.shape[-1]) == x.shape[-1]
+            p_add, s_add, amap = skip_share
+            c_h, gs = x.shape[-1], self.in_channels // self.norm1.num_groups
+            gamma, beta = self.norm1._f32("weight"), self.norm1._f32("bias")
+
+            def conv1():
+                g1 = b.groupnorm(x, gamma[:c_h], beta[:c_h], c_h // gs, self.norm1.eps, True, name="norm1+silu")
+                return g1, b.conv(g1, self._half_pack(self.conv1, b.dtype, 0, c_h), self.conv1._f32("bias"), row_bias=temb_proj,
+                                  addend=p_add, addend_map=amap, name="conv1")
+
+            def shortcut():
+                return b.conv(x, self._half_pack(self.conv_shortcut, b.dtype, 0, c_h), self.conv_shortcut._f32("bias"), name="conv_shortcut")
+            conv2_kw = {"addend": s_add, "addend_map": amap}
+        else:
+            def conv1():
+                g1 = self.norm1.emit(b, x, silu=True, x2=x2, name="norm1+silu")
+                return g1, self.conv1.emit(b, g1, row_bias=temb_proj, name="conv1")
+
+            def shortcut():
+                return self.conv_shortcut.emit(b, x, x2=x2, name="conv_shortcut")
+            conv2_kw = {}
+
         def main_chain():
-            g1 = self.norm1.emit(b, x, silu=True, x2=x2, name="norm1+silu")
-            h = self.conv1.emit(b, g1, row_bias=temb_proj, name="conv1")
+            g1, h = conv1()
             b.free(g1)
             g2 = self.norm2.emit(b, h, silu=True, name="norm2+silu")
             b.free(h)
@@ -199,11 +239,11 @@
                 par.lane()
                 g2 = main_chain()
                 par.lane()
-                sc = self.conv_shortcut.emit(b, x, x2=x2, name="conv_shortcut")
+                sc = shortcut()
         else:
             g2 = main_chain()
-            sc = self.conv_shortcut.emit(b, x, x2=x2, name="conv_shortcut")
-        out = self.conv2.emit(b, g2, residual=sc, name="conv2", **({} if out is None else {"out": out}))
+            sc = shortcut()
+        out = self.conv2.emit(b, g2, residual=sc, name="conv2", **conv2_kw, **({} if out is None else {"out": out}))
         b.free(g2)
         if sc is not x:
             b.free(sc)
diff --git a/mv_ldm_amd/mvunet.py b/mv_ldm_amd/mvunet.py
--- a/mv_ldm_amd/mvunet.py
+++ b/mv_ldm_amd/mvunet.py
@@ -318,6 +318,19 @@
         self.skips = skips
 
 
+class _PrefixSkips(list):
+
+    def __init__(self, skips, partials=None):
+        super().__init__(skips)
+        self.partials = partials or {}
+
+
+class _SkipShare:
+
+    def __init__(self, view, full, index):
+        self.view, self.full, self.index = view, full, index
+
+
 class MultiViewUNet(Denoiser, _PackMixin):
     def __init__(self, cfg: MultiViewUNetCfg, in_channels: int, out_channels: int):
         super().__init__(cfg)
@@ -369,7 +382,7 @@
         return cond_state is None
 
     def emit(self, b: Builder, x_in, timesteps, groups: Sequence[int], out: Optional[torch.Tensor] = None,
-             dup: Optional[tuple] = None, prefix_only: bool = False, tail: Optional[tuple] = None):
+             dup: Optional[tuple] = None, prefix_only: bool = False, tail: Optional[tuple] = None, partial_rows: int = 0):
         u = self.unet
         n_img = x_in.shape[0]
         assert n_img == sum(groups)
@@ -380,6 +393,11 @@
             const = (dup[2], dup[3]) if os.environ.get("MVLDM_CFG_SHARE", "1") != "1a" else None
         n_src = n_img if dup is None else int(dup[0])
         shared = dup is not None
+        skip_share = os.environ.get("MVLDM_SKIP_SHARE", "1") != "0" and not os.environ.get("MVLDM_IGEMM_TILE")
+        up_resnets = [r for blk in u.up_blocks for r in blk.resnets]
+
+        def consumer(i):
+            return up_resnets[len(up_resnets) - 1 - i] if i < len(up_resnets) else None
         lo, hi = (n_src, n_img) if const is not None else (0, n_src)
         with b.scope("time"):
             t_emb = u.time_proj.emit(b, timesteps, dtype=b.dtype)
@@ -394,9 +412,30 @@
             full = b.empty(n_img, *shape_of, dtype=b.dtype)
             return {"out": full[lo:hi]}, full
 
+        amap = []
+
+        def addend_map():
+            if not amap:
+                n_c, n_d = const[0].numel(), n_img - n_src
+                ar = torch.arange(n_img, dtype=torch.int32, device=b.device)
+                m = torch.empty(n_img, dtype=torch.int32, device=b.device)
+                m[const[0].to(b.device).long()] = ar[:n_c]
+                m[dup[1].to(b.device).long()] = n_c + ar[:n_d]
+                m[n_src:] = n_c + ar[:n_d]
+                b.keep.append(m)
+                amap.append(m)
+            return amap[0]
+
         def resnet(r, name, h, skip=None, **kw):
             with b.scope(name):
                 tp_ = tproj[id(r)]
+                if isinstance(skip, _SkipShare):
+                    assert h.shape[0] == n_img and not shared
+                    p_add, s_add = const[1].partials[skip.index]
+                    b.keep.extend([p_add, s_add])
+                    n_c = const[0].numel()
+                    r.emit_skip_partials(b, skip.view, h.shape[-1], p_add[n_c:], s_add[n_c:])
+                    return r.emit(b, h, None, temb_proj=tp_, skip_share=(p_add, s_add, addend_map()), **kw)
                 return r.emit(b, h, None, x2=skip, temb_proj=tp_[lo:hi] if shared else tp_, **kw)
 
         def sd_attn(attn, name, h, **kw):
@@ -415,16 +454,35 @@
         def expand(h):
             nonlocal shared
             if prefix_only:
-                raise _PrefixDone(list(skips))
+                partials = {}
+                if skip_share and partial_rows > 0:
+                    for i, t in enumerate(skips):
+                        r = consumer(i)
+                        if t is h or r is None or r.skip_split(t.shape[-1]) is None:
+                            continue
+                        p_st, s_st = (torch.empty(n_img + partial_rows, *t.shape[1:3], r.conv1.out_channels, dtype=torch.float32, device=b.device)
+                                      for _ in range(2))
+                        b.keep.extend([p_st, s_st])
+                        with b.scope(f"skip{i}.partials"):
+                            r.emit_skip_partials(b, t, r.in_channels - t.shape[-1], p_st[:n_img], s_st[:n_img])
+                        partials[i] = (p_st, s_st)
+                raise _PrefixDone(_PrefixSkips(skips, partials))
             if not shared:
                 return h
             shared = False
             with b.scope("cfg_share"):
                 for i, t in enumerate(skips):
                     full = fulls[id(t)]
+                    r = consumer(i)
+                    if (skip_share and const is not None and full is not fulls[id(h)] and r is not None
+                            and r.skip_split(t.shape[-1]) is not None and i in getattr(const[1], "partials", {})
+                            and const[1].partials[i][0].shape[0] == const[0].numel() + n_img - n_src):
+                        skips[i] = _SkipShare(t, full, i)
+                        continue
                     fill(full, i, f"skip{i}")
                     skips[i] = full
-                assert id(h) in fulls and any(fulls[id(h)] is t for t in skips), "the running activation at a multi-view block is a skip"
+                assert id(h) in fulls and any(fulls[id(h)] is t for t in skips if not isinstance(t, _SkipShare)), \
+                    "the running activation at a multi-view block is a skip"
                 return fulls[id(h)]
 
         def mv(blocks, idx, name, h, **kw):
@@ -449,7 +507,7 @@
                 tail = None
             return self._emit_body(b, u, h, skips, fulls, dest, resnet, sd_attn, mv, expand, out, groups, tail)
         except _PrefixDone as done:
-            return done.skips
+            return done.skips if isinstance(done.skips, _PrefixSkips) else _PrefixSkips(done.skips)
 
     def _emit_body(self, b, u, h, skips, fulls, dest, resnet, sd_attn, mv, expand, out, groups, tail=None):
         live_mv = None
@@ -512,7 +570,7 @@
                 skip = skips.pop()
                 nh = resnet(r, f"up{lvl}.resnets.{i}", h, skip)
                 b.free(h)
-                b.free(skip)
+                b.free(skip.full if isinstance(skip, _SkipShare) else skip)
                 h = nh
                 if has_attn:
                     h2 = sd_attn(blk.attentions[i], f"up{lvl}.attentions.{i}", h)
diff --git a/mv_ldm_amd/ops.py b/mv_ldm_amd/ops.py
--- a/mv_ldm_amd/ops.py
+++ b/mv_ldm_amd/ops.py
@@ -166,7 +166,7 @@
 
 def igemm_desc(src0, src1, pw: PackedWeight, dst, *, n_img, h_in, w_in, h_out, w_out, stride=1, pad=None, upsample=False,
                bias=None, row_bias=None, residual=None, epilogue=L.EPI_NONE, out_scale=1.0, ws=None, splitk=0,
-               tile=0, into=None) -> L.IgemmDesc:
+               tile=0, into=None, addend=None, addend_map=None) -> L.IgemmDesc:
     d = L.IgemmDesc() if into is None else into
     c0 = src0.shape[-1]
     c1 = 0 if src1 is None else src1.shape[-1]
@@ -185,6 +185,11 @@
     n_dst = pw.n_out // 2 if epilogue == L.EPI_GEGLU else pw.n_out
     d.dst_ld = 0 if dst.shape[-1] == n_dst else dst.shape[-1]
     d.k_order = pw.k_order
+    assert (addend is None) == (addend_map is None), "addend and addend_map come together"
+    if addend is not None:
+        assert addend.dtype == torch.float32 and addend.is_contiguous() and addend.numel() == addend.shape[0] * h_out * w_out * pw.n_out
+        assert addend_map.dtype == torch.int32 and addend_map.is_contiguous() and addend_map.numel() == n_img
+    d.addend, d.addend_map = ptr(addend), ptr(addend_map)
     if (tile & 63) == 15:
         use_skinny(d, pw)
     if ws is not None:
@@ -197,7 +202,8 @@
 
 
 def conv2d(x: torch.Tensor, pw: PackedWeight, bias=None, *, x2=None, stride=1, pad=None, upsample=False, row_bias=None,
-           residual=None, epilogue=L.EPI_NONE, out_dtype=None, out_scale=1.0, splitk=0, tile=0, out=None, dst=None) -> torch.Tensor:
+           residual=None, epilogue=L.EPI_NONE, out_dtype=None, out_scale=1.0, splitk=0, tile=0, out=None, dst=None,
+           addend=None, addend_map=None) -> torch.Tensor:
     assert x.is_cuda and x.is_contiguous() and (x2 is None or x2.is_contiguous())
     n, h, w, _ = x.shape
     pad = (pw.ksize // 2) if pad is None else pad
@@ -214,11 +220,11 @@
         assert out.is_contiguous() and out.numel() == n * ho * wo * n_dst and out.dtype == (out_dtype or x.dtype)
         out = out.view(n, ho, wo, n_dst)
     scratch = None
-    if splitk != 1:
+    if splitk != 1 and addend is None:
         scratch = workspace(min(16 * n * ho * wo * pw.n_pad * 4, 256 << 20), x.device)
     d = igemm_desc(x, x2, pw, out, n_img=n, h_in=h, w_in=w, h_out=ho, w_out=wo, stride=stride, pad=pad,
                    upsample=upsample, bias=bias, row_bias=row_bias, residual=residual, epilogue=epilogue,
-                   out_scale=out_scale, ws=scratch, splitk=splitk, tile=tile)
+                   out_scale=out_scale, ws=scratch, splitk=splitk, tile=tile, addend=addend, addend_map=addend_map)
     L.check(L.load().mvldm_igemm_fwd(C.byref(d), stream()))
     return out
 
diff --git a/mv_ldm_amd/pipeline.py b/mv_ldm_amd/pipeline.py
--- a/mv_ldm_amd/pipeline.py
+++ b/mv_ldm_amd/pipeline.py
@@ -209,7 +209,7 @@
                 t_ctx = torch.zeros(b * v_c, dtype=torch.int64, device=dev)
                 cb.gather_rows(unet_in, x_ctx, src_index=ctx_rows, name="context rows")
                 with cb.scope("unet_ctx"):
-                    const_skips = den.emit(cb, x_ctx, t_ctx, [1] * (b * v_c), prefix_only=True)
+                    const_skips = den.emit(cb, x_ctx, t_ctx, [1] * (b * v_c), prefix_only=True, partial_rows=n_unc)
                 cb.keep.extend([x_ctx, t_ctx, *const_skips])
                 const_plan = cb.finalize()
                 dup = (n_cond, cond_img, ctx_rows, const_skips)
diff --git a/mv_ldm_amd/plan.py b/mv_ldm_amd/plan.py
--- a/mv_ldm_amd/plan.py
+++ b/mv_ldm_amd/plan.py
@@ -149,7 +149,8 @@
             L.check(L.load().mvldm_op_run(C.byref(op), torch.cuda.current_stream().cuda_stream))
 
     def conv(self, x, pw: PackedWeight, bias=None, *, x2=None, stride=1, pad=None, upsample=False, row_bias=None,
-             residual=None, epilogue=L.EPI_NONE, out_dtype=None, out_scale=1.0, out=None, name="conv", splitk=0, tile=0):
+             residual=None, epilogue=L.EPI_NONE, out_dtype=None, out_scale=1.0, out=None, name="conv", splitk=0, tile=0,
+             addend=None, addend_map=None):
         n, h, w, c0 = x.shape
         c1 = 0 if x2 is None else x2.shape[-1]
         pad = (pw.ksize // 2) if pad is None else pad
@@ -157,6 +158,8 @@
         n_dst = pw.n_out // 2 if epilogue == L.EPI_GEGLU else pw.n_out
         if out is None:
             out = self.empty(n, ho, wo, n_dst, dtype=out_dtype or x.dtype)
+        if addend is not None:
+            splitk = 1
         ws = self.splitk_ws() if splitk != 1 else None
         if tile == 0 and _PIN_TILE() and x.dtype != torch.float32 and pw.k_order == 1:
             tile, splitk = _PIN_TILE(), 1
@@ -164,9 +167,10 @@
         k_real = pw.ksize * pw.ksize * (c0 + c1)
         es = x.element_size()
         nbytes = (pw.n_out * k_real + n * h * w * (c0 + c1)) * es + m * n_dst * out.element_size() \
-            + (m * n_dst * es if residual is not None else 0)
+            + (m * n_dst * es if residual is not None else 0) + (m * n_dst * 4 if addend is not None else 0)
         self._igemm(x, x2, pw, bias, row_bias, residual, out, ws, name, 2.0 * m * pw.n_out * k_real, nbytes, h_out=ho, w_out=wo,
-                    stride=stride, pad=pad, upsample=upsample, epilogue=epilogue, out_scale=out_scale, splitk=splitk, tile=tile)
+                    stride=stride, pad=pad, upsample=upsample, epilogue=epilogue, out_scale=out_scale, splitk=splitk, tile=tile,
+                    **({} if addend is None else {"addend": addend, "addend_map": addend_map}))
         return out
 
     def _igemm(self, x, x2, pw, bias, row_bias, residual, out, ws, name, flops, nbytes, *, h_out, w_out, tile=0, **desc):
@@ -188,7 +192,8 @@
             own = self.__dict__.get("_own_ptrs", ())
             self.__dict__.setdefault("_tune_srcs", {})[len(self.ops)] = tuple(t if (t is not None and t.data_ptr() in own) else None
                                                                               for t in (x, x2))
-        self._emit(op, name, flops, nbytes, (x, x2, pw.data, pw._skinny if (tile & 63) == 15 else None, bias, row_bias, residual, out))
+        self._emit(op, name, flops, nbytes, (x, x2, pw.data, pw._skinny if (tile & 63) == 15 else None, bias, row_bias, residual, out,
+                                             desc.get("addend"), desc.get("addend_map")))
 
     def small_launch(self, rows: int, n_out: int) -> bool:
         limit = int(os.environ.get("MVLDM_PAR_ROWS", "0"))
@@ -451,7 +456,7 @@
 def _igemm_signature(d) -> tuple:
     return (d.n_img, d.h_in, d.w_in, d.h_out, d.w_out, d.c0, d.c1, d.ksize, d.stride, d.pad, d.upsample, d.n_out, d.n_pad,
             d.k_pad, d.epilogue, d.act_dtype, d.dst_dtype, d.k_order, d.dst_ld, bool(d.residual), bool(d.row_bias),
-            bool(d.bias), d.splitk, d.workspace_bytes)
+            bool(d.bias)) + (("addend",) if d.addend else ()) + (d.splitk, d.workspace_bytes)
 
 
 _SMALL_ROWS = int(os.environ.get("MVLDM_TUNE_SMALL_ROWS", "64"))
@@ -641,6 +646,7 @@
     d.dst = off(d.dst, i0 * px_out * (d.dst_ld or n_dst) * ds)
     d.residual = off(d.residual, i0 * px_out * n_dst * es)
     d.row_bias = off(d.row_bias, i0 * d.row_bias_ld * 4)
+    d.addend_map = off(d.addend_map, i0 * 4)
     d.n_img = n
     d.tile, d.splitk = 0, 0
     return q
```
